# sharckhai/drsa-audio

Measured on AMD Instinct MI355X. Metric: explained samples/sec (LRP+DRSA k=4), higher is better.
Workload: dtype fp32; 1 GPU; GTZAN-128 HeatmapGenerator: LRP (WSquare/Gamma/Epsilon name map) + DRSA subspace heatmaps, K=4 at layer j=7 (conv3 block, d=64), sorted info dict; global_batch=512, per_gpu_batch=512, input=128x128 log-mel, parallelism=data-parallel x1 (no collective on the data path), launch=single process, one_device_rehearsal=False

## Files before the change

### drsa_audio_amd/_capi.py

```python
from __future__ import annotations

import ctypes as C
import os
from typing import Optional

import torch

_HERE = os.path.dirname(os.path.abspath(__file__))
LIB_PATH = os.environ.get("DRSA_AMD_LIB") or os.path.join(_HERE, "lib", "libdrsa_amd.so")

_lib: Optional[C.CDLL] = None

_vp, _fp, _ip = C.c_void_p, C.c_void_p, C.c_void_p
_i64, _i32, _sz, _f32, _f64 = C.c_int64, C.c_int, C.c_size_t, C.c_float, C.c_double

SIGNATURES = {
    "drsa_amd_last_error": (C.c_char_p, []),
    "drsa_amd_version": (_i32, []),
    "drsa_amd_drsa_workspace_bytes": (_sz, [_i64, _i32, _i32]),
    "drsa_amd_drsa_slab_floats": (_sz, [_i32, _i32]),
    "drsa_amd_drsa_partial": (_i32, [_fp, _fp, _i64, _i32, _i32, _fp, _fp, _vp, _sz, _vp]),
    "drsa_amd_drsa_finish": (_i32, [_fp, _i64, _i32, _i32, _fp, _fp, _fp, _i32, _ip, _vp]),
    "drsa_amd_drsa_step": (_i32, [_fp, _fp, _i64, _i32, _i32, _fp, _fp, _fp, _vp, _sz, _vp]),
    "drsa_amd_drsa_fused_supported": (_i32, [_i32, _i32]),
    "drsa_amd_drsa_fused_step": (_i32, [_fp, _fp, _i64, _i32, _i32, _fp, _i64, _fp, _fp, _fp, _fp, _vp, _sz, _vp]),
    "drsa_amd_drsa_fused_step_counted": (_i32, [_fp, _fp, _i64, _i32, _i32, _fp, _i64, _fp, _fp, _fp, _ip, _fp, _vp,
                                                _sz, _vp]),
    "drsa_amd_drsa_finish_counted": (_i32, [_fp, _i64, _i32, _i32, _fp, _fp, _fp, _ip, _vp]),
    "drsa_amd_drsa_coop_status": (_i32, [_vp, _i64, _i32, _i32, _ip, _vp]),
    "drsa_amd_debug_coop_spin_budget": (_i32, [C.c_longlong]),
    "drsa_amd_drsa_objective": (_i32, [_fp, _fp, _i64, _i32, _i32, _fp, _fp, _vp, _sz, _vp]),
    "drsa_amd_drsa_run": (_i32, [_fp, _fp, _i64, _i32, _i32, _fp, _fp, _i32, _fp, _ip, _vp, _sz, _i32, _vp]),
    "drsa_amd_drsa_run_multi": (_i32, [_i32, _vp, _i32, _i32, _vp]),
    "drsa_amd_drsa_run_batched": (_i32, [_i32, _vp, _i32, _i32, _i32, _vp]),
    "drsa_amd_drsa_partial_bf16": (_i32, [_vp, _vp, _i64, _i32, _i32, _fp, _fp, _vp, _sz, _vp]),
    "drsa_amd_drsa_partial_f16": (_i32, [_vp, _vp, _i64, _i32, _i32, _fp, _fp, _vp, _sz, _vp]),
    "drsa_amd_drsa_any_supported": (_i32, [_i32, _i32]),
    "drsa_amd_drsa_any_slab_floats": (_sz, [_i32, _i32]),
    "drsa_amd_drsa_any_workspace_bytes": (_sz, [_i64, _i32, _i32]),
    "drsa_amd_drsa_any_partial": (_i32, [_fp, _fp, _i64, _i32, _i32, _fp, _fp, _vp, _sz, _vp]),
    "drsa_amd_drsa_any_finish": (_i32, [_fp, _i64, _i32, _i32, _fp, _fp, _fp, _i32, _ip, _vp]),
    "drsa_amd_drsa_any_finish_counted": (_i32, [_fp, _i64, _i32, _i32, _fp, _fp, _fp, _ip, _vp]),
    "drsa_amd_drsa_any_step": (_i32, [_fp, _fp, _i64, _i32, _i32, _fp, _fp, _fp, _vp, _sz, _vp]),
    "drsa_amd_drsa_any_objective": (_i32, [_fp, _fp, _i64, _i32, _i32, _fp, _fp, _vp, _sz, _vp]),
    "drsa_amd_drsa_any_run": (_i32, [_fp, _fp, _i64, _i32, _i32, _fp, _fp, _i32, _fp, _ip, _vp, _sz, _i32, _vp]),
    "drsa_amd_polar": (_i32, [_fp, _i32, _fp, _ip, _vp]),
    "drsa_amd_subspace_relevances_workspace_bytes": (_sz, [_i64, _i64, _i32, _i32]),
    "drsa_amd_subspace_relevances": (_i32, [_fp, _fp, _i64, _i64, _i32, _i32, _fp, _fp, _vp, _sz, _vp]),
    "drsa_amd_prca_workspace_bytes": (_sz, [_i64, _i32]),
    "drsa_amd_prca_partial": (_i32, [_fp, _fp, _i64, _i32, _fp, _vp, _sz, _vp]),
    "drsa_amd_prca_finish": (_i32, [_fp, _i64, _i32, _fp, _vp]),
    "drsa_amd_syevj_workspace_bytes": (_sz, [_i32]),
    "drsa_amd_syevj": (_i32, [_fp, _i32, _fp, _fp, _ip, _vp, _sz, _vp]),
    "drsa_amd_conv_weight_floats": (_sz, [_i32, _i32, _i32]),
    "drsa_amd_conv_fwd": (_i32, [_fp, _fp, _fp, _fp, _fp, _vp, _fp, _i32, _i32, _i32, _i32, _i32, _i32, _i32, _vp]),
    "drsa_amd_conv_weight_bf16_elems": (_sz, [_i32, _i32, _i32]),
    "drsa_amd_conv_fwd_has_kernel": (_i32, [_i32, _i32, _i32, _i32, _i32, _i32]),
    "drsa_amd_conv_fwd_bf16": (_i32, [_fp, _vp, _fp, _fp, _fp, _vp, _fp, _i32, _i32, _i32, _i32, _i32, _i32, _i32,
                                      _vp]),
    "drsa_amd_conv_bwd": (_i32, [_fp, _vp, _fp, _fp, _fp, _fp, _i32, _i32, _i32, _i32, _i32, _i32, _i32, _i32,
                                 _i32, _f32, _vp]),
    "drsa_amd_conv_bwd_bf16": (_i32, [_fp, _vp, _vp, _fp, _fp, _fp, _i32, _i32, _i32, _i32, _i32, _i32, _i32, _i32,
                                      _i32, _f32, _vp]),
    "drsa_amd_conv_fwd_den_ring": (_i32, [_fp, _fp, _fp, _fp, _fp, _vp, _fp, _i32, _i32, _i32, _i32, _i32, _vp]),
    "drsa_amd_conv_bwd_den_ring": (_i32, [_fp, _vp, _vp, _i32, _fp, _fp, _fp, _fp, _i32, _i32, _i32, _i32, _i32, _i32,
                                          _i32, _i32, _f32, _vp]),
    "drsa_amd_conv_bwd_den_map": (_i32, [_fp, _vp, _i32, _vp, _i32, _fp, _fp, _fp, _i32, _i32, _i32, _i32, _i32, _i32,
                                         _i32, _i32, _f32, _vp]),
    "drsa_amd_conv_bwd_has_kernel_pw": (_i32, [_i32, _i32, _i32, _i32, _i32]),
    "drsa_amd_conv_bwd_has_kernel_bf16_pw": (_i32, [_i32, _i32, _i32, _i32]),
    "drsa_amd_conv_bwd_bf16_pw": (_i32, [_fp, _vp, _i32, _vp, _fp, _fp, _fp, _i32, _i32, _i32, _i32, _i32, _i32,
                                         _i32, _i32, _f32, _vp]),
    "drsa_amd_conv_bwd_has_kernel_bf16": (_i32, [_i32, _i32, _i32, _i32, _i32]),
    "drsa_amd_convk_supported": (_i32, [_i32, _i32, _i32, _i32]),
    "drsa_amd_convk_weight_floats": (_sz, [_i32, _i32, _i32, _i32, _i32]),
    "drsa_amd_convk_fwd": (_i32, [_fp, _fp, _fp, _fp, _fp, _fp, _i32, _i32, _i32, _i32, _i32, _i32, _i32, _i32, _vp]),
    "drsa_amd_convk_bwd": (_i32, [_fp, _fp, _fp, _fp, _fp, _i32, _i32, _i32, _i32, _i32, _i32, _i32, _i32, _i32,
                                  _i32, _i32, _f32, _vp]),
    "drsa_amd_linear_fwd": (_i32, [_fp, _fp, _fp, _fp, _fp, _i32, _i32, _i32, _vp]),
    "drsa_amd_linear_bwd": (_i32, [_fp, _ip, _i32, _fp, _i32, _i32, _f32, _fp, _fp, _i32, _fp, _i32, _f32, _fp,
                                   _i32, _i32, _i32, _vp]),
    "drsa_amd_linear_rule_fwd": (_i32, [_fp, _fp, _fp, _fp, _fp, _fp, _fp, _fp, _fp, _fp, _fp, _i32, _i32, _i32, _i32,
                                        _vp]),
    "drsa_amd_linear_rule_bwd": (_i32, [_fp, _ip, _i32, _fp, _i32, _fp, _fp, _i32, _i32, _f32, _fp, _fp, _fp, _i32,
                                        _i32, _fp, _i32, _f32, _fp, _i32, _i32, _i32, _vp]),
    "drsa_amd_projection_residual": (_i32, [_fp, _i32, _fp, _vp]),
    "drsa_amd_projection_fwd": (_i32, [_fp, _fp, _fp, _fp, _fp, _fp, _vp, _i32, _i32, _i32, _i32, _i32, _vp]),
    "drsa_amd_projection_bwd": (_i32, [_fp, _vp, _fp, _fp, _fp, _fp, _fp, _fp, _fp, _i32, _i32, _i32, _i32, _i32,
                                       _f32, _f32, _i32, _vp]),
    "drsa_amd_projection_fwd_multi": (_i32, [_fp, _fp, _fp, _ip, _i32, _fp, _fp, _fp, _vp, _i32, _i32, _i32, _i32,
                                             _i32, _vp]),
    "drsa_amd_projection_bwd_multi": (_i32, [_fp, _vp, _fp, _fp, _fp, _fp, _fp, _fp, _ip, _i32, _fp, _i32, _i32, _i32,
                                             _i32, _i32, _f32, _f32, _i32, _vp]),
    "drsa_amd_ab_split": (_i32, [_fp, _fp, _fp, _fp, _fp, _i32, _i32, _i64, _f32, _vp]),
    "drsa_amd_ab_combine": (_i32, [_fp, _fp, _f32, _f32, _fp, _fp, _fp, _i32, _i32, _i64, _i32, _f32, _vp]),
    "drsa_amd_relevance_post": (_i32, [_fp, _fp, _fp, _fp, _i32, _i32, _i64, _i32, _f32, _vp]),
    "drsa_amd_first_layer_bwd": (_i32, [_fp, _vp, _fp, _fp, _i32, _i32, _i32, _i32, _i32, _vp]),
    "drsa_amd_first_layer_den": (_i32, [_fp, _fp, _fp, _i32, _i32, _i32, _i32, _vp]),
    "drsa_amd_first_layer_zbox_maps": (_i32, [_fp, _fp, _fp, _fp, _fp, _fp, _fp, _fp, _i32, _i32, _i32, _vp]),
    "drsa_amd_first_layer_zbox_den": (_i32, [_fp, _vp, _fp, _fp, _fp, _i32, _i32, _i32, _i32, _vp]),
    "drsa_amd_first_layer_zbox_bwd": (_i32, [_fp, _vp, _fp, _fp, _fp, _fp, _fp, _i32, _i32, _i32, _i32, _i32, _vp]),
    "drsa_amd_heatmap_sort": (_i32, [_fp, _i32, _i32, _i32, _i32, _fp, _fp, _fp, _fp, _vp, _vp]),
    "drsa_amd_maxpool_capture": (_i32, [_fp, _fp, _fp, _vp, _fp, _i32, _i32, _i32, _i32, _i32, _i32, _vp]),
    "drsa_amd_relevance_unpool": (_i32, [_fp, _vp, _i32, _i32, _i32, _i32, _i32, _i32, _i32, _fp, _vp]),
    "drsa_amd_avgpool_fwd": (_i32, [_fp, _fp, _i32, _i32, _i32, _i32, _i32, _i32, _vp]),
    "drsa_amd_avgpool_bwd": (_i32, [_fp, _fp, _fp, _fp, _i32, _i32, _f32, _f32, _fp, _fp, _i32, _i32, _i32, _i32,
                                    _i32, _i32, _i32, _vp]),
    "drsa_amd_drsa_vectors": (_i32, [_fp, _fp, _vp, _ip, _i32, _i32, _i32, _i32, _i32, _i32, _i32, _i32, _fp, _fp,
                                     _vp]),
    "drsa_amd_normalize_workspace_bytes": (_sz, []),
    "drsa_amd_normalize_vectors": (_i32, [_fp, _i64, _i32, _fp, _vp, _sz, _vp]),
    "drsa_amd_normalize_sumsq": (_i32, [_fp, _i64, _vp, _sz, _fp, _vp]),
    "drsa_amd_normalize_scale": (_i32, [_fp, _i64, _i32, _fp, _i32, _i64, _fp, _vp]),
    "drsa_amd_logmel_smem_bytes": (_i32, [_i32, _i32, _i32, _i32, _i32]),
    "drsa_amd_logmel": (_i32, [_fp, _i64, _i64, _i32, _i64, _i32, _i32, _i32, _i32, _i32, _i32, _fp, _ip, _ip, _ip,
                               _fp, _i32, _i32, _i32, _f32, _f32, _fp, _vp]),
    "drsa_amd_stft_mel_phase": (_i32, [_fp, _i64, _i64, _i32, _i32, _i32, _i32, _i32, _i32, _i32, _fp, _ip, _ip, _ip,
                                       _fp, _i32, _i32, _fp, _fp, _vp]),
    "drsa_amd_heatmap_mask": (_i32, [_fp, _i64, _i32, _i32, _i32, _i32, _i32, _fp, _i32, _fp, _vp]),
    "drsa_amd_istft_envelope": (_i32, [_fp, _i32, _i32, _i32, _fp]),
    "drsa_amd_mel_to_audio": (_i32, [_fp, _fp, _fp, _i64, _i32, _i32, _i32, _i32, _i32, _i32, _fp, _fp, _fp, _fp,
                                     _vp]),
    "drsa_amd_audio_normalize": (_i32, [_fp, _i64, _i32, _fp, _i64, _i32, _i32, _vp]),
    "drsa_amd_mel_relevance_to_stft": (_i32, [_fp, _fp, _fp, _i64, _i32, _i32, _i32, _i32, _ip, _ip, _ip, _fp, _i32,
                                              _f32, _fp, _vp]),
    "drsa_amd_heatmap_mask_large": (_i32, [_fp, _i64, _i32, _i32, _i32, _i32, _i32, _fp, _i32, _fp, _vp]),
    "drsa_amd_stft_mask_to_audio": (_i32, [_fp, _fp, _i64, _i32, _i32, _i32, _i32, _fp, _fp, _fp, _vp]),
}

class DrsaProblem(C.Structure):
    _fields_ = [("A", _vp), ("C", _vp), ("N", _i64), ("d", _i32), ("K", _i32), ("U_io", _vp), ("U_tmp", _vp),
                ("f_traj", _vp), ("counter", _vp), ("ws", _vp), ("ws_size", _sz), ("dtype", _i32)]


DRSA_OK, DRSA_EINVAL, DRSA_EWORKSPACE, DRSA_EUNSUPPORTED, DRSA_ETIMEOUT = 0, -1, -2, -3, -4

XM_NONE, XM_MUL, XM_SPLIT = 0, 1, 2
POST_NONE, POST_DIV, POST_MASK, POST_DIV_RING = 0, 1, 2, 3
POST_DIV_MAP = 4


class DrsaAmdError(RuntimeError):
    pass


def load(path: str = LIB_PATH) -> C.CDLL:
    global _lib
    if _lib is not None:
        return _lib
    if not os.path.exists(path):
        raise DrsaAmdError(
            f"drsa_amd HIP library not found at {path}; build it with "
            f"`python -m drsa_audio_amd.build` (hipcc, gfx950). There is no CPU fallback.")
    lib = C.CDLL(path)
    for name, (res, args) in SIGNATURES.items():
        fn = getattr(lib, name)
        fn.restype = res
        fn.argtypes = args
    _lib = lib
    return lib


def lib() -> C.CDLL:
    return _lib if _lib is not None else load()


def check(rc: int, what: str = "") -> None:
    if rc != 0:
        msg = lib().drsa_amd_last_error().decode(errors="replace")
        raise DrsaAmdError(f"{what or 'drsa_amd'} failed (rc={rc}): {msg}")


def require_gpu(t: torch.Tensor, name: str, dtype=torch.float32) -> None:
    if not isinstance(t, torch.Tensor):
        raise DrsaAmdError(f"{name}: expected a torch.Tensor on the GPU, got {type(t).__name__}")
    if not t.is_cuda:
        raise DrsaAmdError(f"{name}: tensor must live on the GPU (HIP device); got {t.device}. "
                           "drsa_audio_amd has no CPU path.")
    if dtype is not None and t.dtype != dtype:
        raise DrsaAmdError(f"{name}: expected {dtype}, got {t.dtype}")
    if not t.is_contiguous():
        raise DrsaAmdError(f"{name}: tensor must be contiguous")


def ptr(t: Optional[torch.Tensor]) -> Optional[int]:
    return None if t is None else t.data_ptr()


def stream_ptr(device: Optional[torch.device] = None) -> int:
    return torch.cuda.current_stream(device).cuda_stream


def call(name: str, *args) -> None:
    fn = getattr(lib(), name)
    check(fn(*args), name)
```

### drsa_audio_amd/csrc/conv_bwd_b.hip

```cpp
#include "lrp_conv_inst.h"

#ifndef DRSA_CONV_CIC_BWD32
#define DRSA_CONV_CIC_BWD32 8
#endif
#ifndef DRSA_CONV_CIC_BWD64_32
#define DRSA_CONV_CIC_BWD64_32 8
#endif

CONV_TABLE(kTableBwdB,
    BWD_SET(64, 32, DRSA_CONV_CIC_BWD64_32),
    BWD_SET(32, 32, DRSA_CONV_CIC_BWD32))

#ifdef DRSA_CONV_STAMP
extern "C" int drsa_amd_debug_conv_stamps(void* buf) {
  return (int)hipMemcpyToSymbol(HIP_SYMBOL(drsa_conv::g_conv_stamps), &buf, sizeof(buf));
}
#endif
```

### drsa_audio_amd/csrc/lrp_conv.hip

```cpp
#include "common.h"
#include "lrp_conv.h"
#include "lrp_conv_table.h"

#include <stdlib.h>

#define DRSA_CONV_TABLES(X) \
  X(FwdA) X(FwdB) X(FwdC) X(FwdD) X(FwdE) X(BwdA) X(BwdB) X(BwdC) X(FwdBfA) X(FwdBfB) X(FwdBfC) X(FwdP4) X(BwdBfA) X(BwdBfB)

namespace drsa_conv {
#define DRSA_CONV_DECLARE(T) extern const Table kTable##T;
DRSA_CONV_TABLES(DRSA_CONV_DECLARE)
extern const Table kTableSmall;
}

namespace {
using drsa_conv::Entry;
using namespace drsa_conv;

#define DRSA_CONV_ADDRESS(T) &drsa_conv::kTable##T,
const drsa_conv::Table* kTables[] = {DRSA_CONV_TABLES(DRSA_CONV_ADDRESS)};

int pad32(int c) { return (c + 31) / 32 * 32; }

const Entry* find(int cin_p, int cout_p, int W, int ng, int amode, int epi, int et = 0, int pw = 2) {
  const int wide = W >= kWideW;
  for (const drsa_conv::Table* t : kTables)
    for (int i = 0; i < t->n; ++i) {
      const Entry& e = t->entries[i];
      if (e.cin_p == cin_p && e.cout_p == cout_p && e.ng == ng && e.amode == amode && e.epi == epi && e.et == et &&
          e.pw == pw && e.wide == wide)
        return &e;
    }
  return nullptr;
}

#ifndef DRSA_CONV_SMALL_WG
#define DRSA_CONV_SMALL_WG 512
#endif
const Entry* small_tile(const Entry* e, int H, int W, int batch) {
  if (e->th != 8 || e->tw != 8) return e;
  if ((int64_t)((H + 7) / 8) * ((W + 7) / 8) * batch >= DRSA_CONV_SMALL_WG) return e;
  for (int i = 0; i < drsa_conv::kTableSmall.n; ++i) {
    const Entry& c = drsa_conv::kTableSmall.entries[i];
    if (c.cin_p == e->cin_p && c.cout_p == e->cout_p && c.ng == e->ng && c.amode == e->amode && c.epi == e->epi &&
        c.et == e->et && c.pw == e->pw)
      return &c;
  }
  return e;
}

int launch(const Entry* e0, const ConvArgs& args, int batch, hipStream_t s) {
  DRSA_REQUIRE((int64_t)(args.cin > args.cout ? args.cin : args.cout) * args.H * args.W < ((int64_t)1 << 31),
               "conv: one sample's channels x H x W must stay below 2^31");
  const Entry* e = small_tile(e0, args.H, args.W, batch);
  DRSA_SMEM(e->fn, e->lds);
  const int tiles = ((args.H + e->th - 1) / e->th) * ((args.W + e->tw - 1) / e->tw);
  hipLaunchKernelGGL(e->fn, dim3(tiles, batch), dim3(kThreads), e->lds, s, args);
  DRSA_LAUNCH_CHECK();
  return DRSA_OK;
}

int cin_pad(int cin) { return cin == 1 ? 1 : pad32(cin); }

const Entry* find_fwd(int cin, int cout, int W, int ng, int pool, int bf16) {
  return find(bf16 ? pad32(cin) : cin_pad(cin), pad32(cout), W, ng, A_DENSE, pool ? EPI_FWD_POOL : EPI_FWD_RELU,
              bf16 ? 1 : 0, pool == 2 ? 4 : 2);
}

const Entry* find_bwd(int cin, int cout, int W, int ng, int sparse, int bf16, int pool_w) {
  return find(pad32(cin), pad32(cout), W, ng, sparse ? A_POOLSPARSE : A_DENSE, EPI_BWD, bf16 ? 1 : 0, pool_w);
}

int no_kernel(const char* entry, int cin, int cout, int W, int ng, int sparse, int bf16, const char* pool_key, int pool) {
  drsa::set_error("%s: no kernel for cin=%d cout=%d W=%d ng=%d sparse=%d bf16=%d %s=%d", entry, cin, cout, W, ng, sparse,
                  bf16 ? 1 : 0, pool_key, pool);
  return DRSA_EUNSUPPORTED;
}

struct FwdCall {
  const char* name;
  const float* in;
  const void* wts;
  int bf16;
  const float *bias, *den_map;
  float* out;
  uint8_t* out_amax;
  float* out_den;
  int den_ring_only;
  int B, cin, cout, H, W, ng, pool;
};

int conv_fwd_run(const FwdCall& c, void* stream) {
  const char* n = c.name;
  DRSA_REQUIRE(c.B > 0 && c.H > 0 && c.W > 0, "%s: bad shape", n);
  DRSA_REQUIRE(!c.bf16 || c.cin > 1, "%s: cin = 1 runs on drsa_amd_conv_fwd (fp32 VALU kernel)", n);
  DRSA_REQUIRE(c.ng >= 1 && c.ng <= 3, "%s: ng must be 1..3", n);
  DRSA_REQUIRE(c.H % 2 == 0 && c.W % 2 == 0, "%s: H and W must be even (got %dx%d)", n, c.H, c.W);
  DRSA_REQUIRE(c.pool >= 0 && c.pool <= 2, "%s: pool must be 0 (none), 1 (2x2) or 2 (2x4)", n);
  DRSA_REQUIRE(!c.pool || c.out_amax, "%s: pool needs out_amax", n);
  DRSA_REQUIRE(c.pool || c.W % 4 == 0, "%s: an unpooled output needs W %% 4 == 0 (float4 epilogue; got W=%d)", n, c.W);
  DRSA_REQUIRE(c.pool != 2 || c.W % 4 == 0, "%s: a 2x4 pool needs W %% 4 == 0 (got W=%d)", n, c.W);
  DRSA_REQUIRE(!c.bf16 || ((uintptr_t)c.wts & 15) == 0, "%s: weights must be 16-byte aligned", n);
  ConvArgs a{};
  a.in = c.in; a.wts = reinterpret_cast<const float*>(c.wts); a.bias = c.bias; a.den_map = c.den_map; a.out = c.out;
  a.out_amax = c.out_amax; a.out_den = c.out_den; a.H = c.H; a.W = c.W; a.cin = c.cin; a.cout = c.cout; a.clones = 1;
  a.den_ring_only = c.den_ring_only;
  if (c.cin == 1 && c.pool == 1 && c.W % 8 == 0)
    return drsa_first_conv_pool(a, pad32(c.cout), c.ng, c.B, (hipStream_t)stream);
  const Entry* e = find_fwd(c.cin, c.cout, c.W, c.ng, c.pool, c.bf16);
  if (!e) return no_kernel(n, c.cin, c.cout, c.W, c.ng, 0, c.bf16, "pool", c.pool);
  return launch(e, a, c.B, (hipStream_t)stream);
}

struct BwdCall {
  const char* name;
  const float* g;
  const uint8_t* g_amax;
  int pool_w;
  const void* wts;
  int bf16;
  const float *x, *den, *den_const4;
  int den_shared;
  float* out;
  int Bq, clones, cin, cout, H, W, ng, xmode, post;
  float eps;
};

int conv_bwd_run(const BwdCall& c, void* stream) {
  const char* n = c.name;
  DRSA_REQUIRE(c.Bq > 0 && c.clones > 0 && c.Bq % c.clones == 0, "%s: bad batch/clones", n);
  if (c.bf16) {
    DRSA_REQUIRE(c.ng == 1, "%s: bf16 weights need ng == 1 (the Gamma x-/W- term is for the fp32 first layer)", n);
    DRSA_REQUIRE(c.cin >= 16, "%s: bf16 weights need cin >= 16 (16-channel bf16 chunks)", n);
    DRSA_REQUIRE(((uintptr_t)c.wts & 15) == 0, "%s: bf16 weights must be 16-byte aligned", n);
  } else {
    DRSA_REQUIRE(c.ng >= 1 && c.ng <= 2, "%s: ng must be 1..2", n);
  }
  DRSA_REQUIRE(c.den_const4 || (c.H % 2 == 0 && c.W % 4 == 0),
               "%s: H must be even and W %% 4 == 0 (got %dx%d)", n, c.H, c.W);
  DRSA_REQUIRE(c.xmode == XM_NONE || c.x, "%s: xmode needs x", n);
  DRSA_REQUIRE(c.post == POST_NONE || (c.x && (c.den || c.post == POST_MASK)), "%s: POST_DIV needs x and den", n);
  const int sparse = c.g_amax != nullptr;
  const Entry* e = find_bwd(c.cin, c.cout, c.W, c.ng, sparse, c.bf16, c.pool_w);
  if (!e) return no_kernel(n, c.cin, c.cout, c.W, c.ng, sparse, c.bf16, "pool_w", c.pool_w);
  ConvArgs a{};
  a.in = c.g; a.in_amax = c.g_amax; a.wts = reinterpret_cast<const float*>(c.wts); a.x = c.x; a.den = c.den;
  a.den_const4 = c.den_const4; a.den_shared = c.den_shared; a.out = c.out; a.H = c.H; a.W = c.W; a.cin = c.cin;
  a.cout = c.cout; a.clones = c.clones; a.xmode = c.xmode; a.post = c.post; a.eps = c.eps;
  return launch(e, a, c.Bq, (hipStream_t)stream);
}

}

extern "C" {

size_t drsa_amd_conv_weight_floats(int cin, int cout, int ng) {
  return (size_t)ng * 9 * cin_pad(cin) * pad32(cout);
}

size_t drsa_amd_conv_weight_bf16_elems(int cin, int cout, int ng) {
  return (size_t)ng * 9 * pad32(cin) * pad32(cout);
}

int drsa_amd_conv_fwd_has_kernel(int cin, int cout, int W, int ng, int pool, int bf16) {
  if (cin == 1 && !bf16 && pool == 1) return 1;
  if (pool < 0 || pool > 2 || ng < 1 || ng > 3 || (bf16 && cin == 1)) return 0;
  return find_fwd(cin, cout, W, ng, pool, bf16) != nullptr;
}

int drsa_amd_conv_bwd_has_kernel_bf16(int cin, int cout, int W, int ng, int sparse) {
  if (cin < 16 || ng != 1) return 0;
  return find_bwd(cin, cout, W, ng, sparse, 1, 2) != nullptr;
}

int drsa_amd_conv_bwd_has_kernel_pw(int cin, int cout, int W, int ng, int pool_w) {
  if (cin < 2 || (pool_w != 2 && pool_w != 4) || (pool_w == 4 && (W / 4) % 4 != 0)) return 0;
  return find_bwd(cin, cout, W, ng, 1, 0, pool_w) != nullptr;
}

int drsa_amd_conv_bwd_has_kernel_bf16_pw(int cin, int cout, int W, int pool_w) {
  if (cin < 16 || (pool_w != 2 && pool_w != 4)) return 0;
  return find_bwd(cin, cout, W, 1, 1, 1, pool_w) != nullptr;
}

int drsa_amd_conv_fwd(const float* in, const float* wts, const float* bias, const float* den_map, float* out,
                      uint8_t* out_amax, float* out_den, int B, int cin, int cout, int H, int W, int ng,
                      int pool, void* stream) {
  return conv_fwd_run({"conv_fwd", in, wts, 0, bias, den_map, out, out_amax, out_den, 0, B, cin, cout, H, W, ng, pool},
                      stream);
}

int drsa_amd_conv_fwd_bf16(const float* in, const uint16_t* wts, const float* bias, const float* den_map, float* out,
                           uint8_t* out_amax, float* out_den, int B, int cin, int cout, int H, int W, int ng,
                           int pool, void* stream) {
  return conv_fwd_run({"conv_fwd_bf16", in, wts, 1, bias, den_map, out, out_amax, out_den, 0, B, cin, cout, H, W, ng, pool},
                      stream);
}

int drsa_amd_conv_fwd_den_ring(const float* in, const float* wts, const float* bias, const float* den_map, float* out,
                               uint8_t* out_amax, float* den_ring, int B, int cout, int H, int W, int ng,
                               void* stream) {
  DRSA_REQUIRE(in && wts && den_map && out && out_amax && den_ring, "conv_fwd_den_ring: null pointer");
  DRSA_REQUIRE(B > 0 && H >= 4 && W > 0 && H % 2 == 0 && W % 16 == 0,
               "conv_fwd_den_ring: needs H >= 4 even and W %% 16 == 0 (got %dx%d)", H, W);
  return conv_fwd_run({"conv_fwd_den_ring", in, wts, 0, bias, den_map, out, out_amax, den_ring, 1, B, 1, cout, H, W, ng, 1},
                      stream);
}

int drsa_amd_conv_bwd(const float* g, const uint8_t* g_amax, const float* wts, const float* x, const float* den,
                      float* out, int Bq, int clones, int cin, int cout, int H, int W, int ng, int xmode,
                      int post, float eps, void* stream) {
  return conv_bwd_run({"conv_bwd", g, g_amax, 2, wts, 0, x, den, nullptr, 0, out, Bq, clones, cin, cout, H, W, ng, xmode,
                       post, eps}, stream);
}

int drsa_amd_conv_bwd_bf16(const float* g, const uint8_t* g_amax, const uint16_t* wts, const float* x, const float* den,
                           float* out, int Bq, int clones, int cin, int cout, int H, int W, int ng, int xmode,
                           int post, float eps, void* stream) {
  return conv_bwd_run({"conv_bwd_bf16", g, g_amax, 2, wts, 1, x, den, nullptr, 0, out, Bq, clones, cin, cout, H, W, ng,
                       xmode, post, eps}, stream);
}

int drsa_amd_conv_bwd_bf16_pw(const float* g, const uint8_t* g_amax, int pool_w, const uint16_t* wts, const float* x,
                              const float* den, float* out, int Bq, int clones, int cin, int cout, int H, int W,
                              int xmode, int post, float eps, void* stream) {
  DRSA_REQUIRE(g_amax && (pool_w == 2 || pool_w == 4), "conv_bwd_bf16_pw: needs g_amax and pool_w 2 or 4");
  return conv_bwd_run({"conv_bwd_bf16_pw", g, g_amax, pool_w, wts, 1, x, den, nullptr, 0, out, Bq, clones, cin, cout, H,
                       W, 1, xmode, post, eps}, stream);
}

int drsa_amd_conv_bwd_den_map(const float* g, const uint8_t* g_amax, int pool_w, const void* wts, int wts_bf16,
                              const float* x, const float* den_map, float* out, int Bq, int clones, int cin, int cout,
                              int H, int W, int ng, int xmode, float eps, void* stream) {
  DRSA_REQUIRE(x && den_map, "conv_bwd_den_map: needs x and den_map");
  DRSA_REQUIRE(!g_amax || pool_w == 2 || pool_w == 4, "conv_bwd_den_map: pool_w must be 2 or 4");
  DRSA_REQUIRE(xmode == XM_NONE || xmode == XM_MUL || xmode == XM_SPLIT, "conv_bwd_den_map: bad xmode");
  const bool pool24 = g_amax && pool_w == 4;
  DRSA_REQUIRE(wts_bf16 || !pool24 || ng == 1, "conv_bwd_den_map: fp32 weights need ng 1 under a 2x4 pool (got ng=%d)", ng);
  DRSA_REQUIRE(!pool24 || (W / 4) % 4 == 0, "conv_bwd_den_map: a 2x4 pool-sparse g needs W / 4 %% 4 == 0 (got W=%d)", W);
  return conv_bwd_run({"conv_bwd_den_map", g, g_amax, g_amax ? pool_w : 2, wts, wts_bf16 != 0, x, den_map, nullptr, 1, out,
                       Bq, clones, cin, cout, H, W, ng, xmode, POST_DIV, eps}, stream);
}

int drsa_amd_conv_bwd_den_ring(const float* g, const uint8_t* g_amax, const void* wts, int wts_bf16, const float* x,
                               const float* den_ring, const float* den_const4, float* out, int Bq, int clones, int cin,
                               int cout, int H, int W, int ng, int xmode, float eps, void* stream) {
  DRSA_REQUIRE(x && den_ring && den_const4, "conv_bwd_den_ring: needs x, den_ring and den_const4");
  DRSA_REQUIRE(H >= 2 && W >= 8 && W % 8 == 0,
               "conv_bwd_den_ring: needs pooled H >= 2 and W >= 8, W %% 8 == 0 (got %dx%d)", H, W);
  DRSA_REQUIRE(xmode == XM_NONE || xmode == XM_MUL || xmode == XM_SPLIT, "conv_bwd_den_ring: bad xmode");
  DRSA_REQUIRE(((uintptr_t)den_const4 & 15) == 0, "conv_bwd_den_ring: den_const4 must be 16-byte aligned");
  return conv_bwd_run({"conv_bwd_den_ring", g, g_amax, 2, wts, wts_bf16 != 0, x, den_ring, den_const4, 0, out, Bq, clones,
                       cin, cout, H, W, ng, xmode, POST_DIV_RING, eps}, stream);
}

}
```

### drsa_audio_amd/csrc/lrp_conv_config.h

```cpp
#pragma once
#include <stddef.h>

#ifndef DRSA_CONV_PD_BWD
#define DRSA_CONV_PD_BWD 2
#endif
#ifndef DRSA_CONV_BWD_ES
#define DRSA_CONV_BWD_ES 1
#endif
#ifndef DRSA_CONV_BWD_WPE
#define DRSA_CONV_BWD_WPE 3
#endif
#ifndef DRSA_CONV_PIN_SMALL
#define DRSA_CONV_PIN_SMALL 1
#endif
#ifndef DRSA_CONV_PD_SMALL
#define DRSA_CONV_PD_SMALL 3
#endif
#ifndef DRSA_CONV_SMALL_WPE
#define DRSA_CONV_SMALL_WPE 4
#endif
#ifndef DRSA_CONV_SMALL_ES
#define DRSA_CONV_SMALL_ES 2
#endif
#ifndef DRSA_CONV_PRE_D
#define DRSA_CONV_PRE_D 0
#endif
#ifndef DRSA_CONV_PRE_N
#define DRSA_CONV_PRE_N 64
#endif
#ifndef DRSA_CONV_BF_WPE
#define DRSA_CONV_BF_WPE 2
#endif
#ifndef DRSA_CONV_FWD_WPE_128
#define DRSA_CONV_FWD_WPE_128 3
#endif
#ifndef DRSA_CONV_FWD_WPE_WIDE
#define DRSA_CONV_FWD_WPE_WIDE 3
#endif
#ifndef DRSA_CONV_FWD_WPE
#define DRSA_CONV_FWD_WPE 3
#endif
#ifndef DRSA_CONV_FWD128_TW
#define DRSA_CONV_FWD128_TW 8
#endif

namespace drsa_conv {

constexpr int kThreads = 256;

template <int V, int M>
constexpr int round_up() { return (V + M - 1) / M * M; }

constexpr int halo_stride(int hx, int mw) {
  int r = hx;
  const int want = (mw == 8) ? 16 : 8;
  while (r % 32 != want) ++r;
  return r;
}

enum AMode { A_DENSE = 0, A_POOLSPARSE = 1 };
enum Epi { EPI_FWD_POOL = 0, EPI_FWD_RELU = 1, EPI_BWD = 2 };

constexpr int kWideW = 32;
constexpr int wide_tile_w(int epi, int et, int cin_p, int cout_p, int fwd128_tw = DRSA_CONV_FWD128_TW) {
  if (et != 0) return 32;
  if (epi != EPI_BWD) return cout_p == 128 ? fwd128_tw : cout_p == 64 ? 16 : 32;
  return (cout_p == 64 && cin_p <= 128) || cout_p == 128 ? 16 : 32;
}
constexpr int tile_mw(int tw) { return tw == 8 ? 4 : 8; }

constexpr int XO = 3;

constexpr int bf_stride(int hx) {
  int r = hx;
  while (r % 16 != 8) ++r;
  return r;
}

template <int CIN, int COUT, int TH, int TW, int MW, int CIC, int NG, int AMODE, int EPI, int ET = 0, int PW = 2>
struct ConvCfg {
  static constexpr int CIN_ = CIN, COUT_ = COUT, TH_ = TH, TW_ = TW, MW_ = MW, CIC_ = CIC, NG_ = NG;
  static constexpr int AMODE_ = AMODE, EPI_ = EPI;
  static constexpr bool BF = ET == 1;
  static constexpr int HY = TH + 2, HX = TW + 2;
  static constexpr int HXB = bf_stride(HX);
  static constexpr size_t bf_halo_floats = (size_t)2 * HY * HXB * 4;
  static constexpr size_t bf_w_floats = (size_t)NG * 9 * 2 * COUT * 4;
  static constexpr int RS = halo_stride(HX + XO, MW);
  static constexpr int PLANE_RAW = HY * RS;
  static constexpr int PLANE = PLANE_RAW + ((PLANE_RAW % 32) == 0 ? 4 : 0);
  static constexpr int MTW = 2 * MW;
  static constexpr int MTH = 32 / MTW;
  static constexpr int MTX = TW / MTW;
  static constexpr int MT = (TH / MTH) * MTX;
  static constexpr int NT = COUT / 32;
  static constexpr int WM = MT >= 4 ? 4 : MT;
  static constexpr int WN = (4 / WM) < NT ? (4 / WM) : NT;
  static constexpr int MPW = MT / WM;
  static constexpr int NPW = NT / WN;
  static constexpr int KC = 9 * CIC;
  static constexpr int KCP = round_up<KC, 2>();
  static constexpr int NCHUNK = CIN / CIC;
  static constexpr int TWP = (TW == 32) ? 48 : TW;
  static constexpr bool SMALL_BWD = EPI == EPI_BWD && NG == 1 && CIC <= 8 && COUT <= 32;
  static constexpr int ES = (EPI == EPI_BWD && WN == 1) ? (SMALL_BWD ? DRSA_CONV_SMALL_ES : DRSA_CONV_BWD_ES) : 1;
  static constexpr int TCH = WN * 32 / ES;
  static constexpr size_t staging_floats =
      BF ? bf_halo_floats + bf_w_floats : (size_t)CIC * PLANE + (size_t)NG * KCP * COUT;
  static constexpr size_t epi_floats = (size_t)TCH * TH * TWP;
  static constexpr size_t lds_floats = staging_floats > epi_floats ? staging_floats : epi_floats;
  static constexpr int WPE = BF ? (COUT <= 64 ? DRSA_CONV_BF_WPE : 1)
                             : (EPI == EPI_BWD && NG == 1) ? (SMALL_BWD ? DRSA_CONV_SMALL_WPE : DRSA_CONV_BWD_WPE)
                             : (EPI != EPI_BWD && CIC <= 8 && COUT <= 32 && NG <= 2 ? DRSA_CONV_FWD_WPE
                                : EPI != EPI_BWD && CIC <= 8 && NG <= 2 && COUT == 64 ? DRSA_CONV_FWD_WPE_WIDE
                                : EPI != EPI_BWD && CIC <= 4 && NG <= 2 && COUT == 128 && TW == 8 ? DRSA_CONV_FWD_WPE_128 : 1);
  static constexpr bool PIN = SMALL_BWD && DRSA_CONV_PIN_SMALL;
  static constexpr int PD = PIN ? DRSA_CONV_PD_SMALL : DRSA_CONV_PD_BWD > 0 && EPI >= EPI_BWD ? DRSA_CONV_PD_BWD : 1;
  static_assert(TH % MTH == 0 && TW % MTW == 0, "tile must be a multiple of the M-tile");
  static_assert(COUT % 32 == 0, "COUT must be padded to 32");
  static_assert(CIN % CIC == 0, "CIN must be a multiple of the chunk");
  static_assert(MT % WM == 0 && NT % WN == 0 && WM * WN <= 4, "wave split");
  static_assert(!BF || (CIC == 16 && (EPI < EPI_BWD ? AMODE == A_DENSE : EPI == EPI_BWD)),
                "bf16: 16-channel chunks; dense forward, or the per-clone backward (dense or pool-sparse g)");
  static_assert(PW == 2 || (PW == 4 && (EPI == EPI_FWD_POOL || (EPI == EPI_BWD && AMODE == A_POOLSPARSE &&
                                                                  (ET == 1 || TW % 16 == 0)))),
                "2x4 pool windows: the forward pool epilogue, or the backward's pool-sparse staging (fp32: "
                "tiles of whole float4 cell groups)");
  static constexpr int PW_ = PW;
};

}
```

### drsa_audio_amd/csrc/lrp_conv_inst.h

```cpp
#pragma once
#include "lrp_conv_kernel.h"
#include "lrp_conv_table.h"

namespace drsa_conv {

template <int... P>
constexpr Entry conv_entry(int wide) {
  static_assert(sizeof...(P) == 11, "CONV_ENTRY takes every ConvCfg parameter");
  constexpr int p[] = {P...};
  return Entry{p[0], p[1], p[2], p[3], p[4], p[5], p[6], p[7], p[8],
               conv3x3_kernel<P...>, ConvCfg<P...>::lds_floats * sizeof(float), p[9], p[10], wide};
}
#define CONV_ENTRY(CIN, COUT, TH, TW, MW, CIC, NG, AM, EP, ET, PW) \
  drsa_conv::conv_entry<CIN, COUT, TH, TW, MW, CIC, NG, AM, EP, ET, PW>(0)
#define CONV_ENTRY_WIDE(CIN, COUT, TH, TW, MW, CIC, NG, AM, EP, ET, PW) \
  drsa_conv::conv_entry<CIN, COUT, TH, TW, MW, CIC, NG, AM, EP, ET, PW>(1)

#define CONV_FAMILY(CIN, COUT, CIC, NG, AM, EP, ET, PW)                                             \
  CONV_ENTRY_WIDE(CIN, COUT, 8, drsa_conv::wide_tile_w(EP, ET, CIN, COUT),                          \
                  drsa_conv::tile_mw(drsa_conv::wide_tile_w(EP, ET, CIN, COUT)), CIC, NG, AM, EP, ET, PW), \
  CONV_ENTRY(CIN, COUT, 8, 8, 4, CIC, NG, AM, EP, ET, PW)

#define FWD_SET_ET(CIN, COUT, CIC, ET)                                                      \
  CONV_FAMILY(CIN, COUT, CIC, 1, drsa_conv::A_DENSE, drsa_conv::EPI_FWD_POOL, ET, 2),        \
  CONV_FAMILY(CIN, COUT, CIC, 2, drsa_conv::A_DENSE, drsa_conv::EPI_FWD_POOL, ET, 2),        \
  CONV_FAMILY(CIN, COUT, CIC, 3, drsa_conv::A_DENSE, drsa_conv::EPI_FWD_POOL, ET, 2),        \
  CONV_FAMILY(CIN, COUT, CIC, 1, drsa_conv::A_DENSE, drsa_conv::EPI_FWD_RELU, ET, 2),        \
  CONV_FAMILY(CIN, COUT, CIC, 2, drsa_conv::A_DENSE, drsa_conv::EPI_FWD_RELU, ET, 2),        \
  CONV_FAMILY(CIN, COUT, CIC, 3, drsa_conv::A_DENSE, drsa_conv::EPI_FWD_RELU, ET, 2)
#define FWD_SET(CIN, COUT, CIC) FWD_SET_ET(CIN, COUT, CIC, 0)
#define FWD_SET_BF(CIN, COUT) FWD_SET_ET(CIN, COUT, 16, 1)

#define FWD_SET_P4(CIN, COUT, CIC, ET)                                                      \
  CONV_FAMILY(CIN, COUT, CIC, 1, drsa_conv::A_DENSE, drsa_conv::EPI_FWD_POOL, ET, 4),        \
  CONV_FAMILY(CIN, COUT, CIC, 2, drsa_conv::A_DENSE, drsa_conv::EPI_FWD_POOL, ET, 4),        \
  CONV_FAMILY(CIN, COUT, CIC, 3, drsa_conv::A_DENSE, drsa_conv::EPI_FWD_POOL, ET, 4)

#define BWD_SET(CIN, COUT, CIC)                                                             \
  CONV_FAMILY(CIN, COUT, CIC, 1, drsa_conv::A_DENSE, drsa_conv::EPI_BWD, 0, 2),              \
  CONV_FAMILY(CIN, COUT, CIC, 2, drsa_conv::A_DENSE, drsa_conv::EPI_BWD, 0, 2),              \
  CONV_FAMILY(CIN, COUT, CIC, 1, drsa_conv::A_POOLSPARSE, drsa_conv::EPI_BWD, 0, 2),         \
  CONV_FAMILY(CIN, COUT, CIC, 2, drsa_conv::A_POOLSPARSE, drsa_conv::EPI_BWD, 0, 2)

#define BWD_SET_BF(CIN, COUT)                                                               \
  CONV_FAMILY(CIN, COUT, 16, 1, drsa_conv::A_DENSE, drsa_conv::EPI_BWD, 1, 2),               \
  CONV_FAMILY(CIN, COUT, 16, 1, drsa_conv::A_POOLSPARSE, drsa_conv::EPI_BWD, 1, 2)
#define BWD_SET_BF_P4(CIN, COUT) CONV_FAMILY(CIN, COUT, 16, 1, drsa_conv::A_POOLSPARSE, drsa_conv::EPI_BWD, 1, 4)

#define CONV_TABLE(NAME, ...)                                                                     \
  namespace drsa_conv {                                                                           \
  static const Entry NAME##_e[] = {__VA_ARGS__};                                                  \
  extern const Table NAME = {NAME##_e, (int)(sizeof(NAME##_e) / sizeof(NAME##_e[0]))};            \
  }

}
```

### drsa_audio_amd/csrc/lrp_conv_kernel.h

```cpp
#pragma once
#include "common.h"
#include "lrp_conv.h"
#include "lrp_conv_config.h"
#include "lrp_conv_mfma.h"
#include "lrp_conv_stage.h"
#include "lrp_conv_stage_bf.h"

#include <type_traits>

namespace drsa_conv {

#ifdef DRSA_CONV_STAMP
static __device__ unsigned long long* g_conv_stamps;
#endif

__device__ const float g_zero_bias3[3 * 128] = {};

template <int CIN, int COUT, int TH, int TW, int MW, int CIC, int NG, int AMODE, int EPI, int ET = 0, int PW = 2>
__global__ __launch_bounds__(kThreads) __attribute__((amdgpu_waves_per_eu(ConvCfg<CIN, COUT, TH, TW, MW, CIC, NG, AMODE, EPI, ET, PW>::WPE))) void conv3x3_kernel(ConvArgs a) {
  using Cfg = ConvCfg<CIN, COUT, TH, TW, MW, CIC, NG, AMODE, EPI, ET, PW>;
  constexpr int HY = Cfg::HY, HX = Cfg::HX, RS = Cfg::RS, PLANE = Cfg::PLANE;
  constexpr int MTH = Cfg::MTH, MTW = Cfg::MTW, MTX = Cfg::MTX;
  constexpr int WM = Cfg::WM, MPW = Cfg::MPW, NPW = Cfg::NPW;
  constexpr int KC = Cfg::KC, KCP = Cfg::KCP;

  extern __shared__ __attribute__((aligned(16))) float smem[];
#ifdef DRSA_CONV_STAMP
  constexpr bool kStamp = EPI == EPI_BWD && CIN == 32 && COUT == 32 && AMODE == A_POOLSPARSE && ET == 0;
  unsigned long long* const stp = kStamp && g_conv_stamps && threadIdx.x == 0
                                      ? g_conv_stamps + ((size_t)blockIdx.y * gridDim.x + blockIdx.x) * 16 : nullptr;
#define CONV_STAMP(slot) do { if (stp) stp[(slot)] = __builtin_amdgcn_s_memtime(); } while (0)
#else
#define CONV_STAMP(slot) do {} while (0)
#endif
  CONV_STAMP(0);
  float* halo = smem;
  float* wl = smem + (Cfg::BF ? Cfg::bf_halo_floats : (size_t)CIC * PLANE);

  const int tid = threadIdx.x, lane = lane_id(), w = wave_id();
  const int H = a.H, W = a.W;
  const int tiles_x = (W + TW - 1) / TW;
  const int tile_id = blockIdx.x, bq = blockIdx.y;
  const int ty0 = (tile_id / tiles_x) * TH;
  const int tx0 = (tile_id % tiles_x) * TW;
  const int bs = bq / a.clones;
  const int wm = w % WM, wn = w / WM;
  const bool active = w < WM * Cfg::WN;
  const int h = lane >> 5;

  int pix_off[MPW], pix_y[MPW], pix_x[MPW];
#pragma unroll
  for (int u = 0; u < MPW; ++u) {
    const int mt = wm * MPW + u;
    const int p = lane & 31, win = p >> 2, sub = p & 3;
    pix_y[u] = (mt / MTX) * MTH + 2 * (win / MW) + (sub >> 1);
    pix_x[u] = (mt % MTX) * MTW + 2 * (win % MW) + (sub & 1);
    pix_off[u] = Cfg::BF ? (h * HY + pix_y[u]) * Cfg::HXB + pix_x[u] : pix_y[u] * RS + pix_x[u] + XO;
  }

  f32x16 acc[NG][MPW][NPW];
#pragma unroll
  for (int g = 0; g < NG; ++g)
#pragma unroll
    for (int u = 0; u < MPW; ++u)
#pragma unroll
      for (int v = 0; v < NPW; ++v)
#pragma unroll
        for (int r = 0; r < 16; ++r) acc[g][u][v][r] = 0.f;

  constexpr int TWP = Cfg::TWP, TCH = Cfg::TCH;
  constexpr int NV4 = TCH * TH * TW / 4;
  constexpr int V4T = (NV4 + kThreads - 1) / kThreads;
  constexpr int NCELL = TCH * (TH / 2) * (TW / 2);
  constexpr int CT = (NCELL + kThreads - 1) / kThreads;
  float* T = smem;
  constexpr int ES = Cfg::ES;
  static_assert(ES == 1 || ES == 2 || ES == 4, "epilogue split must be 1, 2 or 4");
  auto stage = [&](int v, auto valfn, int sub = 0) {
    __syncthreads();
    if (active) {
#pragma unroll
      for (int u = 0; u < MPW; ++u)
#pragma unroll
        for (int r = 0; r < 16; ++r) {
          const int cf = (r & 3) + 8 * (r >> 2) + 4 * h;
          if constexpr (ES == 1) {
            T[((wn * 32 + cf) * TH + pix_y[u]) * TWP + pix_x[u]] = valfn(u, r);
          } else {
            if ((r >> (ES == 2 ? 3 : 2)) == sub) T[((cf - TCH * sub) * TH + pix_y[u]) * TWP + pix_x[u]] = valfn(u, r);
          }
        }
    }
    __syncthreads();
  };
  auto gch = [&](int cl, int v) { return ((cl >> 5) * NPW + v) * 32 + (cl & 31); };
  auto gchs = [&](int cl, int v, int sub) { return ES == 1 ? gch(cl, v) : v * 32 + sub * TCH + cl; };
  typename std::conditional<Cfg::BF, StagerBF<Cfg>, Stager<Cfg>>::type stg;
  stg.load(a, 0, tid, ty0, tx0, bq, bs);
  CONV_STAMP(11);
  for (int chunk = 0; chunk + (EPI == EPI_BWD ? 1 : 0) < Cfg::NCHUNK; ++chunk) {
    __syncthreads();
    if (chunk == 0) CONV_STAMP(9);
    if constexpr (Cfg::BF) stg.store(halo, wl, tid, ty0, tx0);
    else stg.store(halo, wl, tid);
    if (chunk == 0) CONV_STAMP(10);
    __syncthreads();
    CONV_STAMP(1 + 2 * chunk);
    if (chunk + 1 < Cfg::NCHUNK) stg.load(a, (chunk + 1) * CIC, tid, ty0, tx0, bq, bs);
    if (!active) continue;
    if constexpr (Cfg::BF)
      mfma_chunk_bf<Cfg>(reinterpret_cast<const uint4*>(halo), reinterpret_cast<const uint4*>(wl), pix_off, lane, wn, acc);
    else
      mfma_chunk<Cfg, Cfg::PD>(halo, wl, pix_off, lane, wn, acc);
    CONV_STAMP(2 + 2 * chunk);
  }
  constexpr int Q = TH * TW / 4, CS = kThreads / Q;
  static_assert(kThreads % Q == 0, "float4 groups per tile must divide the block");
  const int cl0 = tid / Q, rem = tid % Q;
  const int py = rem / (TW / 4), px = (rem % (TW / 4)) * 4;
  const bool pix_ok = ty0 + py < H && tx0 + px < W;
  const int HW = H * W;
  const size_t pix = pix_ok ? (size_t)(ty0 + py) * W + tx0 + px : 0;
  const float* xs = a.x ? a.x + (size_t)bs * a.cout * HW + pix : nullptr;
  const float* ds = a.den ? a.den + (a.den_shared ? (size_t)0 : (size_t)bs * a.cout * HW) + pix : nullptr;
  float* oqp = a.out + (size_t)bq * a.cout * HW + pix;
  const bool need_x = a.xmode != XM_NONE || a.post != POST_NONE;
  const bool mul_x = a.xmode != XM_NONE, split_x = a.xmode == XM_SPLIT;
  const bool ring = a.post == POST_DIV_RING && a.den_const4;
  const bool post_div = a.post == POST_DIV || ring, post_any = a.post != POST_NONE;
  const float* xsrc = xs ? xs : oqp;
  const float* dsrc = (ds && post_div && !ring) ? ds : xsrc;
  const float eps = a.eps;
  const bool on_ring = !pix_ok || ty0 + py == 0 || ty0 + py == H - 1 || tx0 + px == 0 || tx0 + px + 4 >= W;
  const bool use_c4 = ring && !on_ring;
  const int ring_n = 2 * W + 8 * (H - 2);
  const int Y = ty0 + py, X = tx0 + px;
  const int ring_i = !pix_ok ? 0 : Y == 0 ? X : Y == H - 1 ? W + X : 2 * W + (Y - 1) * 8 + (X == 0 ? 0 : 4);
  const float* rsrc = ring ? a.den + (size_t)bs * a.cout * ring_n + ring_i : dsrc;
  const size_t dstride = ring ? (size_t)ring_n : (size_t)HW;
  const unsigned upix = (unsigned)pix;
  float* const obase = a.out + (size_t)bq * a.cout * HW;
  const float* const xbase = a.x ? a.x + (size_t)bs * a.cout * HW : obase;
  auto epi_loads = [&](int v, int sub, float4 (&xk)[V4T], float4 (&dk)[V4T], bool lx = true, bool ld = true,
                       int i0 = 0, int i1 = -1) {
    if (i1 < 0) i1 = V4T;
#pragma unroll
    for (int it = i0; it < i1; ++it) {
      const int cl = cl0 + it * CS;
      const int co = gchs(cl, v, sub);
      const bool ok = cl < TCH && co < a.cout;
      const int coc = ok ? co : 0;
      if (lx) xk[it] = *reinterpret_cast<const float4*>(xbase + (upix + (unsigned)coc * (unsigned)HW));
      if (ld) dk[it] = *reinterpret_cast<const float4*>(use_c4 ? a.den_const4 + (size_t)coc * 4 : rsrc + coc * dstride);
    }
  };
  constexpr int kPreN = DRSA_CONV_PRE_N < V4T ? DRSA_CONV_PRE_N : V4T;
  float4 pre_x[V4T], pre_d[V4T];
  if constexpr (EPI == EPI_BWD) {
    __syncthreads();
    if constexpr (Cfg::BF) stg.store(halo, wl, tid, ty0, tx0);
    else stg.store(halo, wl, tid);
    __syncthreads();
    CONV_STAMP(2 * Cfg::NCHUNK - 1);
    epi_loads(0, 0, pre_x, pre_d, true, DRSA_CONV_PRE_D, 0, kPreN);

    if (active) {
      if constexpr (Cfg::BF)
        mfma_chunk_bf<Cfg>(reinterpret_cast<const uint4*>(halo), reinterpret_cast<const uint4*>(wl), pix_off, lane, wn,
                           acc);
      else
        mfma_chunk<Cfg, Cfg::PD>(halo, wl, pix_off, lane, wn, acc);
    }
    CONV_STAMP(2 * Cfg::NCHUNK);
  }

  auto pool_cells = [&](auto pwc, auto&& fn) {
    constexpr int PWc = decltype(pwc)::value;
    constexpr int CW = TW / PWc, NC = TCH * (TH / 2) * CW;
    const int H2 = H >> 1, W2 = W / PWc;
#pragma unroll
    for (int it = 0; it < CT; ++it) {
      const int i = tid + it * kThreads;
      if (i < NC) {
        const int cl = i / ((TH / 2) * CW), rem = i % ((TH / 2) * CW);
        const int cy = rem / CW, cx = rem % CW;
        fn(it, cl, cy, cx, (ty0 >> 1) + cy, tx0 / PWc + cx, H2, W2);
      }
    }
  };
#pragma unroll
  for (int v = 0; v < NPW; ++v) {
    if constexpr (EPI == EPI_FWD_POOL || EPI == EPI_FWD_RELU) {
      const float* bb = a.bias ? a.bias : g_zero_bias3;
      float b0[16], b1[16], b2[16];
#pragma unroll
      for (int r = 0; r < 16; ++r) {
        const int co = gch(wn * 32 + (r & 3) + 8 * (r >> 2) + 4 * h, v);
        const bool cok = co < a.cout;
        const float x0 = bb[co], x1 = bb[COUT + co], x2 = bb[2 * COUT + co];
        b0[r] = cok ? x0 : 0.f;
        b1[r] = cok ? x1 : 0.f;
        b2[r] = cok ? x2 : 0.f;
      }
      stage(v, [&](int u, int r) {
        const float z = acc[0][u][v][r] + b0[r];
        float y = z > 0.f ? z : 0.f;
        if (z != z) y = z;
        return y;
      });
      int am_keep[CT];
      if constexpr (EPI == EPI_FWD_POOL) {
        auto pass0 = [&](auto pwc) {
          constexpr int PWc = decltype(pwc)::value;
          pool_cells(pwc, [&](int it, int cl, int cy, int cx, int qy, int qx, int H2, int W2) {
            const int co = gch(cl, v);
            const float* t = T + (cl * TH + 2 * cy) * TWP + PWc * cx;
            int am = 0;
            float m = t[0];
#pragma unroll
            for (int s4 = 1; s4 < 2 * PWc; ++s4) {
              const float yv = t[(s4 / PWc) * TWP + s4 % PWc];
              if (yv > m || (yv != yv && m == m)) { m = yv; am = s4; }
            }
            am_keep[it] = am;
            if (co < a.cout && qy < H2 && qx < W2) {
              const size_t o = (size_t)bq * a.cout * H2 * W2 + (unsigned)((co * H2 + qy) * W2 + qx);
              a.out[o] = m;
              a.out_amax[o] = (uint8_t)am;
            }
          });
        };
        if constexpr (PW == 4) {
#pragma unroll
          for (int it = 0; it < CT; ++it) am_keep[it] = 0;
          pass0(std::integral_constant<int, 4>{});
        } else {
          const int H2 = H >> 1, W2 = W >> 1;
#pragma unroll
          for (int it = 0; it < CT; ++it) {
            const int i = tid + it * kThreads;
            am_keep[it] = 0;
            if (i < NCELL) {
              const int cl = i / ((TH / 2) * (TW / 2)), rem = i % ((TH / 2) * (TW / 2));
              const int cy = rem / (TW / 2), cx = rem % (TW / 2);
              const int co = gch(cl, v);
              const int qy = (ty0 >> 1) + cy, qx = (tx0 >> 1) + cx;
              const float* t = T + (cl * TH + 2 * cy) * TWP + 2 * cx;
              const float yy[4] = {t[0], t[1], t[TWP], t[TWP + 1]};
              int am = 0;
              float m = yy[0];
#pragma unroll
              for (int s4 = 1; s4 < 4; ++s4)
                if (yy[s4] > m || (yy[s4] != yy[s4] && m == m)) { m = yy[s4]; am = s4; }
              am_keep[it] = am;
              if (co < a.cout && qy < H2 && qx < W2) {
                const size_t o = (size_t)bq * a.cout * H2 * W2 + (unsigned)((co * H2 + qy) * W2 + qx);
                a.out[o] = m;
                a.out_amax[o] = (uint8_t)am;
              }
            }
          }
        }
      } else {
#pragma unroll
        for (int it = 0; it < V4T; ++it) {
          const int i = tid + it * kThreads;
          if (i < NV4) {
            const int cl = i / (TH * TW / 4), rem = i % (TH * TW / 4);
            const int py = rem / (TW / 4), px = (rem % (TW / 4)) * 4;
            const int co = gch(cl, v);
            if (co < a.cout && ty0 + py < H && tx0 + px < W) {
              const float4 val = *reinterpret_cast<const float4*>(T + (cl * TH + py) * TWP + px);
              *reinterpret_cast<float4*>(a.out + (size_t)bq * a.cout * H * W + (unsigned)((co * H + ty0 + py) * W + tx0 + px)) = val;
            }
          }
        }
      }
      if (a.out_den && a.den_map) {
        if constexpr (EPI == EPI_FWD_POOL) {
          auto gather_map = [&](auto pwc) {
            constexpr int PWc = decltype(pwc)::value;
            pool_cells(pwc, [&](int it, int cl, int, int, int qy, int qx, int H2, int W2) {
              const int co = gch(cl, v);
              const int am = am_keep[it];
              if (co < a.cout && qy < H2 && qx < W2)
                a.out_den[(size_t)bq * a.cout * H2 * W2 + (unsigned)((co * H2 + qy) * W2 + qx)] =
                    a.den_map[(unsigned)((co * H + 2 * qy + am / PWc) * W + PWc * qx + am % PWc)];
            });
          };
          if constexpr (PW == 4) {
            gather_map(std::integral_constant<int, 4>{});
          } else {
            const int H2 = H >> 1, W2 = W >> 1;
#pragma unroll
            for (int it = 0; it < CT; ++it) {
              const int i = tid + it * kThreads;
              if (i < NCELL) {
                const int cl = i / ((TH / 2) * (TW / 2)), rem = i % ((TH / 2) * (TW / 2));
                const int cy = rem / (TW / 2), cx = rem % (TW / 2);
                const int co = gch(cl, v);
                const int qy = (ty0 >> 1) + cy, qx = (tx0 >> 1) + cx;
                const int am = am_keep[it];
                if (co < a.cout && qy < H2 && qx < W2)
                  a.out_den[(size_t)bq * a.cout * H2 * W2 + (unsigned)((co * H2 + qy) * W2 + qx)] =
                      a.den_map[(unsigned)((co * H + 2 * qy + (am >> 1)) * W + 2 * qx + (am & 1))];
              }
            }
          }
        } else {
#pragma unroll
          for (int it = 0; it < V4T; ++it) {
            const int i = tid + it * kThreads;
            if (i < NV4) {
              const int cl = i / (TH * TW / 4), rem = i % (TH * TW / 4);
              const int py = rem / (TW / 4), px = (rem % (TW / 4)) * 4;
              const int co = gch(cl, v);
              if (co < a.cout && ty0 + py < H && tx0 + px < W)
                *reinterpret_cast<float4*>(a.out_den + (size_t)bq * a.cout * H * W + (unsigned)((co * H + ty0 + py) * W + tx0 + px)) =
                    *reinterpret_cast<const float4*>(a.den_map + (unsigned)((co * H + ty0 + py) * W + tx0 + px));
            }
          }
        }
      } else if (a.out_den) {
        stage(v, [&](int u, int r) {
          if constexpr (NG >= 2) {
            const float z0 = acc[1][u][v][r] + b1[r];
            float z1 = b2[r];
            if constexpr (NG == 3) z1 = acc[2][u][v][r] + b2[r];
            return z0 + z1;
          }
          return acc[0][u][v][r] + b1[r];
        });
        if constexpr (EPI == EPI_FWD_POOL) {
          auto gather_den = [&](auto pwc) {
            constexpr int PWc = decltype(pwc)::value;
            pool_cells(pwc, [&](int it, int cl, int cy, int cx, int qy, int qx, int H2, int W2) {
              const int co = gch(cl, v);
              const int am = am_keep[it];
              if (co < a.cout && qy < H2 && qx < W2)
                a.out_den[(size_t)bq * a.cout * H2 * W2 + (unsigned)((co * H2 + qy) * W2 + qx)] =
                    T[(cl * TH + 2 * cy + am / PWc) * TWP + PWc * cx + am % PWc];
            });
          };
          if constexpr (PW == 4) {
            gather_den(std::integral_constant<int, 4>{});
          } else {
            const int H2 = H >> 1, W2 = W >> 1;
#pragma unroll
            for (int it = 0; it < CT; ++it) {
              const int i = tid + it * kThreads;
              if (i < NCELL) {
                const int cl = i / ((TH / 2) * (TW / 2)), rem = i % ((TH / 2) * (TW / 2));
                const int cy = rem / (TW / 2), cx = rem % (TW / 2);
                const int co = gch(cl, v);
                const int qy = (ty0 >> 1) + cy, qx = (tx0 >> 1) + cx;
                const int am = am_keep[it];
                if (co < a.cout && qy < H2 && qx < W2)
                  a.out_den[(size_t)bq * a.cout * H2 * W2 + (unsigned)((co * H2 + qy) * W2 + qx)] =
                      T[(cl * TH + 2 * cy + (am >> 1)) * TWP + 2 * cx + (am & 1)];
              }
            }
          }
        } else {
#pragma unroll
          for (int it = 0; it < V4T; ++it) {
            const int i = tid + it * kThreads;
            if (i < NV4) {
              const int cl = i / (TH * TW / 4), rem = i % (TH * TW / 4);
              const int py = rem / (TW / 4), px = (rem % (TW / 4)) * 4;
              const int co = gch(cl, v);
              if (co < a.cout && ty0 + py < H && tx0 + px < W) {
                const float4 val = *reinterpret_cast<const float4*>(T + (cl * TH + py) * TWP + px);
                *reinterpret_cast<float4*>(a.out_den + (size_t)bq * a.cout * H * W + (unsigned)((co * H + ty0 + py) * W + tx0 + px)) = val;
              }
            }
          }
        }
      }
    } else {
#pragma unroll
     for (int sub = 0; sub < ES; ++sub) {
      float4 Rk[V4T], xk[V4T], dk[V4T];
      if (v == 0 && sub == 0) {
#pragma unroll
        for (int it = 0; it < kPreN; ++it) xk[it] = pre_x[it];
        epi_loads(v, sub, xk, dk, true, false, kPreN, V4T);
        if (DRSA_CONV_PRE_D) {
#pragma unroll
          for (int it = 0; it < V4T; ++it) dk[it] = pre_d[it];
        } else {
          epi_loads(v, sub, xk, dk, false, true);
        }
      } else {
        epi_loads(v, sub, xk, dk);
      }
      stage(v, [&](int u, int r) { return acc[0][u][v][r]; }, sub);
      if (NG == 1 && a.xmode == XM_MUL && post_div) {
#pragma unroll
        for (int it = 0; it < V4T; ++it) {
          const int cl = cl0 + it * CS;
          const int co = gchs(cl, v, sub);
          const bool ok = cl < TCH && co < a.cout;
          const int clc = ok ? cl : 0, coc = ok ? co : 0;
          const float4 t = *reinterpret_cast<const float4*>(T + (clc * TH + py) * TWP + px);
          const float4 x = xk[it], d = dk[it];
          auto f = [&](float tt, float xx, float dd) {
            const float q = div_nb(xx * tt, stab(dd, eps));
            return (xx > 0.f) ? q : 0.f;
          };
          const float4 R = make_float4(f(t.x, x.x, d.x), f(t.y, x.y, d.y), f(t.z, x.z, d.z), f(t.w, x.w, d.w));
          if (ok && pix_ok) *reinterpret_cast<float4*>(obase + (upix + (unsigned)coc * (unsigned)HW)) = R;
        }
        continue;
      }
#pragma unroll
      for (int it = 0; it < V4T; ++it) {
        const int cl = cl0 + it * CS;
        const int co = gchs(cl, v, sub);
        const int clc = (cl < TCH && co < a.cout) ? cl : 0;
        const float4 t = *reinterpret_cast<const float4*>(T + (clc * TH + py) * TWP + px);
        if (!need_x) xk[it] = make_float4(0.f, 0.f, 0.f, 0.f);
        const float4 x = xk[it];
        auto xm = [&](float xx) { const float m = split_x ? fmaxf(xx, 0.f) : xx; return mul_x ? m : 1.f; };
        Rk[it] = make_float4(xm(x.x) * t.x, xm(x.y) * t.y, xm(x.z) * t.z, xm(x.w) * t.w);
      }
      if constexpr (NG >= 2) {
        if (split_x) {
          stage(v, [&](int u, int r) { return acc[1][u][v][r]; }, sub);
#pragma unroll
          for (int it = 0; it < V4T; ++it) {
            const int cl = cl0 + it * CS;
            const int co = gchs(cl, v, sub);
            const int clc = (cl < TCH && co < a.cout) ? cl : 0;
            const float4 t = *reinterpret_cast<const float4*>(T + (clc * TH + py) * TWP + px);
            const float4 x = xk[it];
            Rk[it].x += fminf(x.x, 0.f) * t.x;
            Rk[it].y += fminf(x.y, 0.f) * t.y;
            Rk[it].z += fminf(x.z, 0.f) * t.z;
            Rk[it].w += fminf(x.w, 0.f) * t.w;
          }
        }
      }
#pragma unroll
      for (int it = 0; it < V4T; ++it) {
        const int cl = cl0 + it * CS;
        const int co = gchs(cl, v, sub);
        const bool ok = cl < TCH && co < a.cout;
        const int coc = ok ? co : 0;
        float4 R = Rk[it];
        const float4 x = xk[it], d = dk[it];
        auto post = [&](float rr, float xx, float dd) {
          const float q = div_nb(rr, stab(dd, eps));
          const float y = post_div ? q : rr;
          return (post_any && !(xx > 0.f)) ? 0.f : y;
        };
        R = make_float4(post(R.x, x.x, d.x), post(R.y, x.y, d.y), post(R.z, x.z, d.z), post(R.w, x.w, d.w));
        if (ok && pix_ok) *reinterpret_cast<float4*>(obase + (upix + (unsigned)coc * (unsigned)HW)) = R;
      }
     }
    }
  }
#ifdef DRSA_CONV_STAMP
  if (stp) {
    stp[13] = __builtin_amdgcn_s_memtime();
    stp[14] = (unsigned long long)__builtin_amdgcn_s_getreg(4 | (31 << 11));
    stp[15] = (unsigned long long)__builtin_amdgcn_s_getreg(20 | (31 << 11));
  }
#endif
#undef CONV_STAMP
}

}
```

### drsa_audio_amd/csrc/lrp_conv_stage.h

```cpp
#pragma once
#include "common.h"
#include "lrp_conv.h"
#include "lrp_conv_config.h"

namespace drsa_conv {

template <class Cfg, int NT_ = kThreads>
struct Stager {
  static constexpr int CIN = Cfg::CIN_, COUT = Cfg::COUT_, TH = Cfg::TH_, TW = Cfg::TW_, CIC = Cfg::CIC_;
  static constexpr int NG = Cfg::NG_, HY = Cfg::HY, HX = Cfg::HX, RS = Cfg::RS, PLANE = Cfg::PLANE;
  static constexpr int KC = Cfg::KC, KCP = Cfg::KCP;
  static constexpr bool DENSE = Cfg::AMODE_ == A_DENSE;
  static constexpr int Q4 = TW / 4, DROWS = CIC * HY;
  static constexpr int DI = (DROWS * Q4 + NT_ - 1) / NT_, DH = (DROWS * 2 + NT_ - 1) / NT_;
  static constexpr int CY = TH / 2 + 2, CX = TW / 2 + 2, Q8 = TW / 8 > 0 ? TW / 8 : 1, SROWS = CIC * CY;
  static constexpr int SI = (SROWS * Q8 + NT_ - 1) / NT_, SH = (SROWS * 2 + NT_ - 1) / NT_;
  static constexpr bool P4 = !DENSE && Cfg::PW_ == 4;
  static constexpr int Q16 = TW / 16 > 0 ? TW / 16 : 1;
  static constexpr int SI4 = (SROWS * Q16 + NT_ - 1) / NT_;
  static constexpr int NI = DENSE ? DI : P4 ? SI4 : SI, NH = DENSE ? DH : SH;
  static constexpr int NWV = NG * KCP * (COUT / 4), WIT = (NWV + NT_ - 1) / NT_;
  float4 st_i[NI];
  uint32_t st_ia[DENSE ? 1 : NI];
  float st_h[NH];
  int st_ha[DENSE ? 1 : NH];
  float4 st_w[WIT];

  __device__ __forceinline__ void load(const ConvArgs& a, int c0, int tid, int ty0, int tx0, int bq, int bs) {
    const int H = a.H, W = a.W, H2 = H >> 1, W2 = W >> 1;
    const int W4 = W >> 2;
    const float* __restrict__ inb = a.in + (size_t)bq * a.cin * (DENSE ? H * W : H2 * (P4 ? W4 : W2));
    const uint8_t* __restrict__ amb = DENSE ? nullptr : a.in_amax + (size_t)bs * a.cin * H2 * (P4 ? W4 : W2);
    if constexpr (P4) {
      const int qy0 = (ty0 >> 1) - 1, cx0 = tx0 >> 2;
#pragma unroll
      for (int it = 0; it < SI4; ++it) {
        const int i = tid + it * NT_;
        const int row = i / Q16, q = i % Q16;
        const int ci = row / CY, ry = row % CY;
        const int cy = qy0 + ry, cx = cx0 + 4 * q, c = c0 + ci;
        const bool ok = i < SROWS * Q16 && cy >= 0 && cy < H2 && c < a.cin && cx < W4;
        const int o = ok ? (c * H2 + cy) * W4 + cx : 0;
        const float4 v = *reinterpret_cast<const float4*>(inb + o);
        const uint32_t am = *reinterpret_cast<const uint32_t*>(amb + o);
        st_i[it] = ok ? v : make_float4(0.f, 0.f, 0.f, 0.f);
        st_ia[it] = ok ? am : 0xffffffffu;
      }
#pragma unroll
      for (int it = 0; it < SH; ++it) {
        const int i = tid + it * NT_;
        const int row = i >> 1, side = i & 1;
        const int ci = row / CY, ry = row % CY;
        const int cy = qy0 + ry, cx = side ? cx0 + TW / 4 : cx0 - 1, c = c0 + ci;
        const bool ok = i < SROWS * 2 && cy >= 0 && cy < H2 && cx >= 0 && cx < W4 && c < a.cin;
        const int o = ok ? (c * H2 + cy) * W4 + cx : 0;
        const float v = inb[o];
        const int am = (int)amb[o];
        st_h[it] = ok ? v : 0.f;
        st_ha[it] = ok ? am : 0xff;
      }
    } else if constexpr (DENSE) {
      if ((W & 3) == 0) {
#pragma unroll
        for (int it = 0; it < DI; ++it) {
          const int i = tid + it * NT_;
          const int row = i / Q4, q = i % Q4;
          const int ci = row / HY, hy = row % HY;
          const int gy = ty0 - 1 + hy, gx = tx0 + 4 * q, c = c0 + ci;
          const bool ok = i < DROWS * Q4 && gy >= 0 && gy < H && c < a.cin && gx < W;
          const int o = ok ? (c * H + gy) * W + gx : 0;
          const float4 v = *reinterpret_cast<const float4*>(inb + o);
          st_i[it] = ok ? v : make_float4(0.f, 0.f, 0.f, 0.f);
        }
      } else {
#pragma unroll
        for (int it = 0; it < DI; ++it) {
          const int i = tid + it * NT_;
          const int row = i / Q4, q = i % Q4;
          const int ci = row / HY, hy = row % HY;
          const int gy = ty0 - 1 + hy, gx = tx0 + 4 * q, c = c0 + ci;
          const bool rok = i < DROWS * Q4 && gy >= 0 && gy < H && c < a.cin;
          float vv[4];
#pragma unroll
          for (int e = 0; e < 4; ++e) {
            const bool ok = rok && gx + e < W;
            const int o = ok ? (c * H + gy) * W + gx + e : 0;
            const float v = inb[o];
            vv[e] = ok ? v : 0.f;
          }
          st_i[it] = make_float4(vv[0], vv[1], vv[2], vv[3]);
        }
      }
#pragma unroll
      for (int it = 0; it < DH; ++it) {
        const int i = tid + it * NT_;
        const int row = i >> 1, side = i & 1;
        const int ci = row / HY, hy = row % HY;
        const int gy = ty0 - 1 + hy, gx = side ? tx0 + TW : tx0 - 1, c = c0 + ci;
        const bool ok = i < DROWS * 2 && gy >= 0 && gy < H && gx >= 0 && gx < W && c < a.cin;
        const int o = ok ? (c * H + gy) * W + gx : 0;
        const float v = inb[o];
        st_h[it] = ok ? v : 0.f;
      }
    } else {
      const int qy0 = (ty0 >> 1) - 1, qx0 = (tx0 >> 1) - 1;
      if ((W2 & 3) == 0) {
#pragma unroll
        for (int it = 0; it < SI; ++it) {
          const int i = tid + it * NT_;
          const int row = i / Q8, q = i % Q8;
          const int ci = row / CY, ry = row % CY;
          const int cy = qy0 + ry, cx = qx0 + 1 + 4 * q, c = c0 + ci;
          const bool ok = i < SROWS * Q8 && 4 * q < TW / 2 && cy >= 0 && cy < H2 && c < a.cin && cx < W2;
          const int o = ok ? (c * H2 + cy) * W2 + cx : 0;
          const float4 v = *reinterpret_cast<const float4*>(inb + o);
          const uint32_t am = *reinterpret_cast<const uint32_t*>(amb + o);
          st_i[it] = ok ? v : make_float4(0.f, 0.f, 0.f, 0.f);
          st_ia[it] = ok ? am : 0x04040404u;
        }
      } else {
#pragma unroll
        for (int it = 0; it < SI; ++it) {
          const int i = tid + it * NT_;
          const int row = i / Q8, q = i % Q8;
          const int ci = row / CY, ry = row % CY;
          const int cy = qy0 + ry, cx = qx0 + 1 + 4 * q, c = c0 + ci;
          const bool rok = i < SROWS * Q8 && 4 * q < TW / 2 && cy >= 0 && cy < H2 && c < a.cin;
          float vv[4];
          uint32_t aa = 0;
#pragma unroll
          for (int e = 0; e < 4; ++e) {
            const bool ok = rok && cx + e < W2 && 4 * q + e < TW / 2;
            const int o = ok ? (c * H2 + cy) * W2 + cx + e : 0;
            const float v = inb[o];
            const uint32_t am = amb[o];
            vv[e] = ok ? v : 0.f;
            aa |= (ok ? am : 4u) << (8 * e);
          }
          st_i[it] = make_float4(vv[0], vv[1], vv[2], vv[3]);
          st_ia[it] = aa;
        }
      }
#pragma unroll
      for (int it = 0; it < SH; ++it) {
        const int i = tid + it * NT_;
        const int row = i >> 1, side = i & 1;
        const int ci = row / CY, ry = row % CY;
        const int cy = qy0 + ry, cx = side ? qx0 + CX - 1 : qx0, c = c0 + ci;
        const bool ok = i < SROWS * 2 && cy >= 0 && cy < H2 && cx >= 0 && cx < W2 && c < a.cin;
        const int o = ok ? (c * H2 + cy) * W2 + cx : 0;
        const float v = inb[o];
        const int am = (int)amb[o];
        st_h[it] = ok ? v : 0.f;
        st_ha[it] = ok ? am : 4;
      }
    }
#pragma unroll
    for (int it = 0; it < WIT; ++it) {
      const int idx = tid + it * NT_;
      const int g = idx / (KCP * (COUT / 4)), rem = idx % (KCP * (COUT / 4));
      const int k = rem / (COUT / 4), c4 = (rem % (COUT / 4)) * 4;
      const bool ok = idx < NWV && k < KC;
      const float4 v = *reinterpret_cast<const float4*>(a.wts + (ok ? ((size_t)g * 9 * CIN + c0 * 9 + k) * COUT + c4 : 0));
      st_w[it] = ok ? v : make_float4(0.f, 0.f, 0.f, 0.f);
    }
  }

  __device__ __forceinline__ static void put_cell(float* halo, int ci, int ry, int rx, float v, int sb) {
    float* d = halo + ci * PLANE + (2 * ry - 1) * RS + 2 * rx - 1 + XO;
    if (ry > 0) *reinterpret_cast<float2*>(d) = make_float2(sb == 0 ? v : 0.f, sb == 1 ? v : 0.f);
    if (ry < CY - 1) *reinterpret_cast<float2*>(d + RS) = make_float2(sb == 2 ? v : 0.f, sb == 3 ? v : 0.f);
  }

  __device__ __forceinline__ static void put_cell4(float* halo, int ci, int ry, int rx, float v, int sb) {
    float* d = halo + ci * PLANE + (2 * ry - 1) * RS + 4 * rx;
    if (ry > 0)
      *reinterpret_cast<float4*>(d) = make_float4(sb == 0 ? v : 0.f, sb == 1 ? v : 0.f, sb == 2 ? v : 0.f, sb == 3 ? v : 0.f);
    if (ry < CY - 1)
      *reinterpret_cast<float4*>(d + RS) =
          make_float4(sb == 4 ? v : 0.f, sb == 5 ? v : 0.f, sb == 6 ? v : 0.f, sb == 7 ? v : 0.f);
  }

  __device__ __forceinline__ void store(float* halo, float* wl, int tid) const {
    if constexpr (P4) {
      static_assert(XO == 3, "P4 cells land on 16-byte aligned columns 4 rx");
#pragma unroll
      for (int it = 0; it < SI4; ++it) {
        const int i = tid + it * NT_;
        if (i < SROWS * Q16) {
          const int row = i / Q16, q = i % Q16;
          const int ci = row / CY, ry = row % CY;
          const float vv[4] = {st_i[it].x, st_i[it].y, st_i[it].z, st_i[it].w};
#pragma unroll
          for (int e = 0; e < 4; ++e)
            put_cell4(halo, ci, ry, 1 + 4 * q + e, vv[e], (int)((st_ia[it] >> (8 * e)) & 0xffu));
        }
      }
#pragma unroll
      for (int it = 0; it < SH; ++it) {
        const int i = tid + it * NT_;
        if (i < SROWS * 2) {
          const int row = i >> 1, side = i & 1;
          put_cell4(halo, row / CY, row % CY, side ? TW / 4 + 1 : 0, st_h[it], st_ha[it]);
        }
      }
    } else if constexpr (DENSE) {
#pragma unroll
      for (int it = 0; it < DI; ++it) {
        const int i = tid + it * NT_;
        if (i < DROWS * Q4) {
          const int row = i / Q4, q = i % Q4;
          const int ci = row / HY, hy = row % HY;
          *reinterpret_cast<float4*>(halo + ci * PLANE + hy * RS + 1 + XO + 4 * q) = st_i[it];
        }
      }
#pragma unroll
      for (int it = 0; it < DH; ++it) {
        const int i = tid + it * NT_;
        if (i < DROWS * 2) {
          const int row = i >> 1, side = i & 1;
          const int ci = row / HY, hy = row % HY;
          halo[ci * PLANE + hy * RS + (side ? HX - 1 : 0) + XO] = st_h[it];
        }
      }
    } else {
#pragma unroll
      for (int it = 0; it < SI; ++it) {
        const int i = tid + it * NT_;
        const int q = i % Q8;
        if (i < SROWS * Q8 && 4 * q < TW / 2) {
          const int row = i / Q8;
          const int ci = row / CY, ry = row % CY;
          const float vv[4] = {st_i[it].x, st_i[it].y, st_i[it].z, st_i[it].w};
#pragma unroll
          for (int e = 0; e < 4; ++e)
            if (4 * q + e < TW / 2) put_cell(halo, ci, ry, 1 + 4 * q + e, vv[e], (int)((st_ia[it] >> (8 * e)) & 0xffu));
        }
      }
#pragma unroll
      for (int it = 0; it < SH; ++it) {
        const int i = tid + it * NT_;
        if (i < SROWS * 2) {
          const int row = i >> 1, side = i & 1;
          put_cell(halo, row / CY, row % CY, side ? CX - 1 : 0, st_h[it], st_ha[it]);
        }
      }
    }
#pragma unroll
    for (int it = 0; it < WIT; ++it) {
      const int idx = tid + it * NT_;
      if (idx < NWV) *reinterpret_cast<float4*>(wl + (size_t)idx * 4) = st_w[it];
    }
  }
};

}
```

### drsa_audio_amd/csrc/lrp_conv_table.h

```cpp
#pragma once
#include "lrp_conv.h"
#include "lrp_conv_config.h"

namespace drsa_conv {

typedef void (*KernFn)(ConvArgs);

struct Entry {
  int cin_p, cout_p, th, tw, mw, cic, ng, amode, epi;
  KernFn fn;
  size_t lds;
  int et = 0;
  int pw = 2;
  int wide = 0;
};

struct Table {
  const Entry* entries;
  int n;
};

}
```

### include/drsa_amd.h

```cpp
#ifndef DRSA_AMD_H
#define DRSA_AMD_H

#include <stddef.h>
#include <stdint.h>

#ifdef __cplusplus
extern "C" {
#endif

#define DRSA_OK 0
#define DRSA_EINVAL (-1)
#define DRSA_EWORKSPACE (-2)
#define DRSA_EUNSUPPORTED (-3)
#define DRSA_ETIMEOUT (-4)

const char* drsa_amd_last_error(void);
int drsa_amd_version(void);


size_t drsa_amd_drsa_workspace_bytes(int64_t N, int d, int K);

size_t drsa_amd_drsa_slab_floats(int d, int K);

int drsa_amd_drsa_partial(const float* A, const float* C, int64_t N, int d, int K, const float* U,
                          float* gs_out, void* workspace, size_t workspace_bytes, void* stream);

int drsa_amd_drsa_finish(const float* gs, int64_t N_total, int d, int K, const float* U, float* U_out,
                         float* f_out, int objective_only, int* iters_out, void* stream);

int drsa_amd_drsa_fused_supported(int d, int K);
int drsa_amd_drsa_fused_step(const float* A, const float* C, int64_t N, int d, int K, const float* gs,
                             int64_t N_total, const float* U, float* U_out, float* f_out, float* gs_out, void* ws,
                             size_t ws_size, void* stream);

int drsa_amd_drsa_fused_step_counted(const float* A, const float* C, int64_t N, int d, int K, const float* gs,
                                     int64_t N_total, const float* U, float* U_out, float* f_traj, int* counter,
                                     float* gs_out, void* ws, size_t ws_size, void* stream);
int drsa_amd_drsa_finish_counted(const float* gs, int64_t N_total, int d, int K, const float* U, float* U_out,
                                 float* f_traj, int* counter, void* stream);

int drsa_amd_drsa_step(const float* A, const float* C, int64_t N, int d, int K, const float* U,
                       float* U_out, float* f_out, void* workspace, size_t workspace_bytes, void* stream);

int drsa_amd_drsa_objective(const float* A, const float* C, int64_t N, int d, int K, const float* U,
                            float* f_out, void* workspace, size_t workspace_bytes, void* stream);

int drsa_amd_drsa_run(const float* A, const float* C, int64_t N, int d, int K, float* U_io, float* U_tmp,
                      int steps, float* f_traj, int* counter, void* workspace, size_t workspace_bytes,
                      int use_graph, void* stream);

int drsa_amd_drsa_coop_status(const void* workspace, int64_t N, int d, int K, int* status_out, void* stream);

int drsa_amd_drsa_any_supported(int d, int K);
size_t drsa_amd_drsa_any_slab_floats(int d, int K);
size_t drsa_amd_drsa_any_workspace_bytes(int64_t N, int d, int K);
int drsa_amd_drsa_any_partial(const float* A, const float* C, int64_t N, int d, int K, const float* U,
                              float* gs_out, void* workspace, size_t workspace_bytes, void* stream);
int drsa_amd_drsa_any_finish(const float* gs, int64_t N_total, int d, int K, const float* U, float* U_out,
                             float* f_out, int objective_only, int* iters_out, void* stream);
int drsa_amd_drsa_any_finish_counted(const float* gs, int64_t N_total, int d, int K, const float* U, float* U_out,
                                     float* f_traj, int* counter, void* stream);
int drsa_amd_drsa_any_step(const float* A, const float* C, int64_t N, int d, int K, const float* U,
                           float* U_out, float* f_out, void* workspace, size_t workspace_bytes, void* stream);
int drsa_amd_drsa_any_objective(const float* A, const float* C, int64_t N, int d, int K, const float* U,
                                float* f_out, void* workspace, size_t workspace_bytes, void* stream);
int drsa_amd_drsa_any_run(const float* A, const float* C, int64_t N, int d, int K, float* U_io, float* U_tmp,
                          int steps, float* f_traj, int* counter, void* workspace, size_t workspace_bytes,
                          int use_graph, void* stream);

int drsa_amd_debug_coop_spin_budget(long long ticks);

int drsa_amd_polar(const float* V, int d, float* U_out, int* iters_out, void* stream);

size_t drsa_amd_subspace_relevances_workspace_bytes(int64_t B, int64_t N, int d, int K);
int drsa_amd_subspace_relevances(const float* act, const float* ctx, int64_t B, int64_t N, int d, int K,
                                 const float* U, float* out, void* workspace, size_t workspace_bytes, void* stream);


size_t drsa_amd_prca_workspace_bytes(int64_t N, int d);

int drsa_amd_prca_partial(const float* A, const float* C, int64_t N, int d, float* slab, void* ws, size_t ws_bytes,
                          void* stream);

int drsa_amd_prca_finish(const float* slab, int64_t N_total, int d, float* M_out, void* stream);

size_t drsa_amd_syevj_workspace_bytes(int d);
int drsa_amd_syevj(const float* M, int d, float* w_out, float* V_out, int* sweeps_out, void* ws, size_t ws_bytes,
                   void* stream);



size_t drsa_amd_conv_weight_floats(int cin, int cout, int ng);

int drsa_amd_conv_fwd(const float* in, const float* wts, const float* bias, const float* den_map, float* out,
                      uint8_t* out_amax, float* out_den, int B, int cin, int cout, int H, int W, int ng,
                      int pool, void* stream);

size_t drsa_amd_conv_weight_bf16_elems(int cin, int cout, int ng);
int drsa_amd_conv_fwd_bf16(const float* in, const uint16_t* wts, const float* bias, const float* den_map, float* out,
                           uint8_t* out_amax, float* out_den, int B, int cin, int cout, int H, int W, int ng,
                           int pool, void* stream);

int drsa_amd_conv_fwd_has_kernel(int cin, int cout, int W, int ng, int pool, int bf16);

int drsa_amd_conv_bwd(const float* g, const uint8_t* g_amax, const float* wts, const float* x, const float* den,
                      float* out, int Bq, int clones, int cin, int cout, int H, int W, int ng, int xmode,
                      int post, float eps, void* stream);

int drsa_amd_conv_bwd_bf16(const float* g, const uint8_t* g_amax, const uint16_t* wts, const float* x, const float* den,
                           float* out, int Bq, int clones, int cin, int cout, int H, int W, int ng, int xmode,
                           int post, float eps, void* stream);
int drsa_amd_conv_bwd_has_kernel_bf16(int cin, int cout, int W, int ng, int sparse);

int drsa_amd_conv_bwd_bf16_pw(const float* g, const uint8_t* g_amax, int pool_w, const uint16_t* wts, const float* x,
                              const float* den, float* out, int Bq, int clones, int cin, int cout, int H, int W,
                              int xmode, int post, float eps, void* stream);
int drsa_amd_conv_bwd_has_kernel_bf16_pw(int cin, int cout, int W, int pool_w);

int drsa_amd_conv_bwd_den_map(const float* g, const uint8_t* g_amax, int pool_w, const void* wts, int wts_bf16,
                              const float* x, const float* den_map, float* out, int Bq, int clones, int cin, int cout,
                              int H, int W, int ng, int xmode, float eps, void* stream);
int drsa_amd_conv_bwd_has_kernel_pw(int cin, int cout, int W, int ng, int pool_w);

int drsa_amd_convk_supported(int kh, int kw, int cin, int cout);
size_t drsa_amd_convk_weight_floats(int kh, int kw, int cin, int cout, int ng);
int drsa_amd_convk_fwd(const float* in, const float* wts, const float* bias, const float* den_map, float* out,
                       float* out_den, int B, int cin, int cout, int H, int W, int kh, int kw, int ng,
                       void* stream);
int drsa_amd_convk_bwd(const float* g, const float* wts, const float* x, const float* den, float* out, int Bq,
                       int clones, int cin, int cout, int H, int W, int kh, int kw, int ng, int xmode, int post,
                       float eps, void* stream);

int drsa_amd_conv_fwd_den_ring(const float* in, const float* wts, const float* bias, const float* den_map, float* out,
                               uint8_t* out_amax, float* den_ring, int B, int cout, int H, int W, int ng,
                               void* stream);
int drsa_amd_conv_bwd_den_ring(const float* g, const uint8_t* g_amax, const void* wts, int wts_bf16, const float* x,
                               const float* den_ring, const float* den_const4, float* out, int Bq, int clones, int cin,
                               int cout, int H, int W, int ng, int xmode, float eps, void* stream);

int drsa_amd_linear_fwd(const float* x, const float* W, const float* bias, float* z_out, float* relu_out, int M,
                        int N, int K, void* stream);

int drsa_amd_linear_bwd(const float* R, const int* seed_cls, int one_hot, const float* z, int relu_mask, int rule_eps,
                        float eps, const float* W, const float* x, int xmode, const float* den, int post,
                        float eps_post, float* out, int M, int Nout, int Kin, void* stream);

int drsa_amd_linear_rule_fwd(const float* x, const float* W, const float* Wp, const float* Wn, const float* bias,
                             const float* bias_p, const float* bias_n, float* z_out, float* relu_out, float* den_p,
                             float* den_n, int x_signed, int M, int N, int K, void* stream);
int drsa_amd_linear_rule_bwd(const float* R, const int* seed_cls, int one_hot, const float* z, int relu_mask,
                             const float* den_p, const float* den_n, int den_bcast, int zsign, float eps,
                             const float* Wp, const float* Wn, const float* x, int xmul, int x_signed,
                             const float* den, int post, float eps_post, float* out, int M, int Nout, int Kin,
                             void* stream);

int drsa_amd_projection_residual(const float* U, int d, float* P, void* stream);

int drsa_amd_projection_fwd(const float* a, const float* U, const float* P, float* h, float* ap, float* pooled,
                            uint8_t* amax, int B, int D, int H, int W, int pool, void* stream);

int drsa_amd_projection_bwd(const float* gp, const uint8_t* amax, const float* ap, const float* h, const float* a,
                            const float* den, const float* U, const float* P, float* G, int B, int D, int H, int W,
                            int K, float eps_proj, float eps_den, int fanout, void* stream);

int drsa_amd_projection_fwd_multi(const float* a, const float* U_tab, const float* P_tab, const int* u_row, int n_u,
                                  float* h, float* ap, float* pooled, uint8_t* amax, int B, int D, int H, int W,
                                  int pool, void* stream);
int drsa_amd_projection_bwd_multi(const float* gp, const uint8_t* amax, const float* ap, const float* h,
                                  const float* a, const float* den, const float* U_tab, const float* P_tab,
                                  const int* u_row, int n_u, float* G, int B, int D, int H, int W, int K,
                                  float eps_proj, float eps_den, int fanout, void* stream);

int drsa_amd_ab_split(const float* g, const float* den_p, const float* den_n, float* gp, float* gn, int Bq,
                      int clones, int64_t n, float eps, void* stream);
int drsa_amd_ab_combine(const float* pos, const float* neg, float alpha, float beta, const float* x, const float* den,
                        float* out, int Bq, int clones, int64_t n, int post, float eps, void* stream);

int drsa_amd_relevance_post(const float* R, const float* x, const float* den, float* out, int Bq, int clones,
                            int64_t n, int post, float eps, void* stream);

int drsa_amd_first_layer_bwd(const float* g, const uint8_t* amax, const float* w2, float* out, int Bq, int clones,
                             int C, int H, int W, void* stream);

int drsa_amd_first_layer_den(const float* w2, const float* b2, float* den, int C, int CI, int H, int W, void* stream);

int drsa_amd_first_layer_zbox_maps(const float* wp, const float* bp, const float* wn, const float* bn,
                                   const float* low_img, const float* high_img, float* zl, float* zh, int C, int H,
                                   int W, void* stream);
int drsa_amd_first_layer_zbox_den(const float* a, const uint8_t* amax, const float* zl, const float* zh, float* den,
                                  int B, int C, int H, int W, void* stream);
int drsa_amd_first_layer_zbox_bwd(const float* g, const uint8_t* amax, const float* wpn, const float* x,
                                  const float* low_img, const float* high_img, float* out, int Bq, int clones, int C,
                                  int H, int W, void* stream);

int drsa_amd_heatmap_sort(const float* hm, int B, int K, int HW, int std_from_sum, float* std_out, float* std_rel,
                          float* sub_out, float* rel, int64_t* mask, void* stream);

typedef struct drsa_amd_problem {
  const float* A;
  const float* C;
  int64_t N;
  int d;
  int K;
  float* U_io;
  float* U_tmp;
  float* f_traj;
  int* counter;
  void* ws;
  size_t ws_size;
  int dtype;
} drsa_amd_problem_t;

int drsa_amd_drsa_partial_bf16(const uint16_t* A, const uint16_t* C, int64_t N, int d, int K, const float* U,
                               float* gs_out, void* ws, size_t ws_size, void* stream);
int drsa_amd_drsa_partial_f16(const uint16_t* A, const uint16_t* C, int64_t N, int d, int K, const float* U,
                              float* gs_out, void* ws, size_t ws_size, void* stream);

int drsa_amd_drsa_run_multi(int P, const drsa_amd_problem_t* probs, int steps, int use_graph, void* stream);

int drsa_amd_drsa_run_batched(int P, const drsa_amd_problem_t* probs, int steps, int blocks, int use_graph,
                              void* stream);

int drsa_amd_logmel_smem_bytes(int n_fft, int hop, int n_mels, int width, int band_nnz);
int drsa_amd_logmel(const float* wav, int64_t n_songs, int64_t song_stride, int chunks_per_song, int64_t chunk_hop,
                    int chunk_len, int n_fft, int hop, int n_mels, int width, int frame0, const float* window,
                    const int* band_lo, const int* band_n, const int* band_off, const float* band_w, int band_nnz,
                    int peak_norm, int clamp, float clamp_min, float log_eps, float* out, void* stream);


int drsa_amd_maxpool_capture(const float* a, const float* den, float* y, uint8_t* amax, float* den_pooled, int B,
                             int C, int H, int W, int ph, int pw, void* stream);

int drsa_amd_relevance_unpool(const float* rel, const uint8_t* amax, int Bq, int clones, int C, int H, int W, int ph,
                              int pw, float* out, void* stream);

int drsa_amd_avgpool_fwd(const float* a, float* y, int B, int C, int H, int W, int ph, int pw, void* stream);

int drsa_amd_avgpool_bwd(const float* R_y, const float* y, const float* a, const float* den, int den_bcast, int rule,
                         float eps_pool, float eps_conv, float* g, float* rel_full, int Bq, int clones, int C, int H,
                         int W, int ph, int pw, void* stream);

int drsa_amd_drsa_vectors(const float* act, const float* rel, const uint8_t* rel_amax, const int* idx, int B, int C,
                          int H, int W, int ph, int pw, int L, int layout, float* A_out, float* C_out, void* stream);

size_t drsa_amd_normalize_workspace_bytes(void);
int drsa_amd_normalize_vectors(const float* v, int64_t n, int d, float* out, void* ws, size_t ws_bytes, void* stream);

int drsa_amd_normalize_sumsq(const float* v, int64_t n, void* ws, size_t ws_bytes, double* sum_out, void* stream);
int drsa_amd_normalize_scale(const float* v, int64_t n, int d, const double* sums, int nsums, int64_t n_total,
                             float* out, void* stream);


int drsa_amd_stft_mel_phase(const float* wav, int64_t n_chunks, int64_t chunk_stride, int chunk_len, int n_fft,
                            int hop, int n_mels, int width, int frame0, int power, const float* window,
                            const int* band_lo, const int* band_n, const int* band_off, const float* band_w,
                            int band_nnz, int peak_norm, float* mel, float* X, void* stream);

int drsa_amd_heatmap_mask(const float* heatmaps, int64_t n_maps, int H, int W, int group, int rank_first,
                          int rank_rest, const float* taps, int k, float* mask, void* stream);

int drsa_amd_istft_envelope(const float* window_host, int n_fft, int hop, int width, float* envelope_host);

int drsa_amd_mel_to_audio(const float* mel, const float* X, const float* mask, int64_t n_src, int C, int n_fft,
                          int hop, int n_mels, int width, int power, const float* window, const float* pinv_t,
                          const float* envelope, float* audio, void* stream);

int drsa_amd_audio_normalize(float* audio, int64_t n_audio, int len, const float* wav, int64_t wav_stride,
                             int wav_len, int C, void* stream);


int drsa_amd_mel_relevance_to_stft(const float* relevance, const float* mel, const float* X, int64_t n_src, int C,
                                   int n_mels, int width, int n_freq, const int* bin_lo, const int* bin_n,
                                   const int* bin_off, const float* bin_w, int bin_nnz, float eps, float* out,
                                   void* stream);

int drsa_amd_heatmap_mask_large(const float* heatmaps, int64_t n_maps, int H, int W, int group, int rank_first,
                                int rank_rest, const float* taps, int k, float* mask, void* stream);

int drsa_amd_stft_mask_to_audio(const float* X, const float* mask, int64_t n_src, int C, int n_fft, int hop,
                                int width, const float* window, const float* envelope, float* audio, void* stream);

#ifdef __cplusplus
}
#endif
#endif
```

Before: 115,300 explained samples/s.

## Process two relevance clones per workgroup in fp32 conv backward

Adds a clone-pair variant of the fp32 small-chunk 3x3 conv backward kernel in which each workgroup stages and computes two clones (DRSA subspace copies) of the same sample. The clones share the weights in LDS, the x/den epilogue loads and the tile setup, and the grid's batch dimension is halved. It is enabled by default for dense inputs when the clone count is even. In exchange it doubles halo and epilogue LDS and the per-wave accumulators, which can lower occupancy, and it halves the number of workgroups.

Measured after the change: 115,300 explained samples/s (median of 2 runs). Within noise of the previous version (-0.0%).

```diff
diff --git a/drsa_audio_amd/_capi.py b/drsa_audio_amd/_capi.py
--- a/drsa_audio_amd/_capi.py
+++ b/drsa_audio_amd/_capi.py
@@ -69,6 +69,7 @@
                                          _i32, _i32, _f32, _vp]),
     "drsa_amd_conv_bwd_has_kernel_pw": (_i32, [_i32, _i32, _i32, _i32, _i32]),
     "drsa_amd_conv_bwd_has_kernel_bf16_pw": (_i32, [_i32, _i32, _i32, _i32]),
+    "drsa_amd_conv_bwd_clones_per_wg": (_i32, [_i32, _i32, _i32, _i32, _i32, _i32, _i32, _i32]),
     "drsa_amd_conv_bwd_bf16_pw": (_i32, [_fp, _vp, _i32, _vp, _fp, _fp, _fp, _i32, _i32, _i32, _i32, _i32, _i32,
                                          _i32, _i32, _f32, _vp]),
     "drsa_amd_conv_bwd_has_kernel_bf16": (_i32, [_i32, _i32, _i32, _i32, _i32]),
diff --git a/drsa_audio_amd/csrc/conv_bwd_b.hip b/drsa_audio_amd/csrc/conv_bwd_b.hip
--- a/drsa_audio_amd/csrc/conv_bwd_b.hip
+++ b/drsa_audio_amd/csrc/conv_bwd_b.hip
@@ -7,9 +7,21 @@
 #define DRSA_CONV_CIC_BWD64_32 8
 #endif
 
+#if DRSA_CONV_PAIR_SPARSE
+#define PAIR_SPARSE(CIN, COUT) , CONV_ENTRY_PAIR(CIN, COUT, drsa_conv::A_POOLSPARSE)
+#else
+#define PAIR_SPARSE(CIN, COUT)
+#endif
+#if DRSA_CONV_PAIR_DENSE
+#define PAIR_DENSE(CIN, COUT) , CONV_ENTRY_PAIR(CIN, COUT, drsa_conv::A_DENSE)
+#else
+#define PAIR_DENSE(CIN, COUT)
+#endif
+
 CONV_TABLE(kTableBwdB,
     BWD_SET(64, 32, DRSA_CONV_CIC_BWD64_32),
-    BWD_SET(32, 32, DRSA_CONV_CIC_BWD32))
+    BWD_SET(32, 32, DRSA_CONV_CIC_BWD32)
+    PAIR_SPARSE(64, 32) PAIR_SPARSE(32, 32) PAIR_DENSE(64, 32) PAIR_DENSE(32, 32))
 
 #ifdef DRSA_CONV_STAMP
 extern "C" int drsa_amd_debug_conv_stamps(void* buf) {
diff --git a/drsa_audio_amd/csrc/lrp_conv.hip b/drsa_audio_amd/csrc/lrp_conv.hip
--- a/drsa_audio_amd/csrc/lrp_conv.hip
+++ b/drsa_audio_amd/csrc/lrp_conv.hip
@@ -22,13 +22,13 @@
 
 int pad32(int c) { return (c + 31) / 32 * 32; }
 
-const Entry* find(int cin_p, int cout_p, int W, int ng, int amode, int epi, int et = 0, int pw = 2) {
+const Entry* find(int cin_p, int cout_p, int W, int ng, int amode, int epi, int et = 0, int pw = 2, int cp = 1) {
   const int wide = W >= kWideW;
   for (const drsa_conv::Table* t : kTables)
     for (int i = 0; i < t->n; ++i) {
       const Entry& e = t->entries[i];
       if (e.cin_p == cin_p && e.cout_p == cout_p && e.ng == ng && e.amode == amode && e.epi == epi && e.et == et &&
-          e.pw == pw && e.wide == wide)
+          e.pw == pw && e.wide == wide && e.cp == cp)
         return &e;
     }
   return nullptr;
@@ -55,7 +55,7 @@
   const Entry* e = small_tile(e0, args.H, args.W, batch);
   DRSA_SMEM(e->fn, e->lds);
   const int tiles = ((args.H + e->th - 1) / e->th) * ((args.W + e->tw - 1) / e->tw);
-  hipLaunchKernelGGL(e->fn, dim3(tiles, batch), dim3(kThreads), e->lds, s, args);
+  hipLaunchKernelGGL(e->fn, dim3(tiles, batch / e->cp), dim3(kThreads), e->lds, s, args);
   DRSA_LAUNCH_CHECK();
   return DRSA_OK;
 }
@@ -69,6 +69,13 @@
 
 const Entry* find_bwd(int cin, int cout, int W, int ng, int sparse, int bf16, int pool_w) {
   return find(pad32(cin), pad32(cout), W, ng, sparse ? A_POOLSPARSE : A_DENSE, EPI_BWD, bf16 ? 1 : 0, pool_w);
+}
+
+const Entry* pick_bwd(int cin, int cout, int W, int ng, int sparse, int bf16, int pool_w, int clones) {
+  const Entry* e = find_bwd(cin, cout, W, ng, sparse, bf16, pool_w);
+  if (!e || bf16 || clones < 2 || clones % 2 != 0) return e;
+  const Entry* p = find(pad32(cin), pad32(cout), W, ng, sparse ? A_POOLSPARSE : A_DENSE, EPI_BWD, 0, pool_w, 2);
+  return p ? p : e;
 }
 
 int no_kernel(const char* entry, int cin, int cout, int W, int ng, int sparse, int bf16, const char* pool_key, int pool) {
@@ -141,7 +148,7 @@
   DRSA_REQUIRE(c.xmode == XM_NONE || c.x, "%s: xmode needs x", n);
   DRSA_REQUIRE(c.post == POST_NONE || (c.x && (c.den || c.post == POST_MASK)), "%s: POST_DIV needs x and den", n);
   const int sparse = c.g_amax != nullptr;
-  const Entry* e = find_bwd(c.cin, c.cout, c.W, c.ng, sparse, c.bf16, c.pool_w);
+  const Entry* e = pick_bwd(c.cin, c.cout, c.W, c.ng, sparse, c.bf16, c.pool_w, c.clones);
   if (!e) return no_kernel(n, c.cin, c.cout, c.W, c.ng, sparse, c.bf16, "pool_w", c.pool_w);
   ConvArgs a{};
   a.in = c.g; a.in_amax = c.g_amax; a.wts = reinterpret_cast<const float*>(c.wts); a.x = c.x; a.den = c.den;
@@ -181,6 +188,11 @@
 int drsa_amd_conv_bwd_has_kernel_bf16_pw(int cin, int cout, int W, int pool_w) {
   if (cin < 16 || (pool_w != 2 && pool_w != 4)) return 0;
   return find_bwd(cin, cout, W, 1, 1, 1, pool_w) != nullptr;
+}
+
+int drsa_amd_conv_bwd_clones_per_wg(int cin, int cout, int W, int ng, int sparse, int bf16, int pool_w, int clones) {
+  const Entry* e = pick_bwd(cin, cout, W, ng, sparse, bf16, pool_w, clones);
+  return e ? e->cp : 1;
 }
 
 int drsa_amd_conv_fwd(const float* in, const float* wts, const float* bias, const float* den_map, float* out,
diff --git a/drsa_audio_amd/csrc/lrp_conv_config.h b/drsa_audio_amd/csrc/lrp_conv_config.h
--- a/drsa_audio_amd/csrc/lrp_conv_config.h
+++ b/drsa_audio_amd/csrc/lrp_conv_config.h
@@ -43,6 +43,18 @@
 #ifndef DRSA_CONV_FWD128_TW
 #define DRSA_CONV_FWD128_TW 8
 #endif
+#ifndef DRSA_CONV_PAIR_SPARSE
+#define DRSA_CONV_PAIR_SPARSE 0
+#endif
+#ifndef DRSA_CONV_PAIR_DENSE
+#define DRSA_CONV_PAIR_DENSE 1
+#endif
+#ifndef DRSA_CONV_PAIR_TW
+#define DRSA_CONV_PAIR_TW 32
+#endif
+#ifndef DRSA_CONV_PAIR_PRE_D
+#define DRSA_CONV_PAIR_PRE_D 2
+#endif
 
 namespace drsa_conv {
 
@@ -77,10 +89,10 @@
   return r;
 }
 
-template <int CIN, int COUT, int TH, int TW, int MW, int CIC, int NG, int AMODE, int EPI, int ET = 0, int PW = 2>
+template <int CIN, int COUT, int TH, int TW, int MW, int CIC, int NG, int AMODE, int EPI, int ET = 0, int PW = 2, int CP = 1>
 struct ConvCfg {
   static constexpr int CIN_ = CIN, COUT_ = COUT, TH_ = TH, TW_ = TW, MW_ = MW, CIC_ = CIC, NG_ = NG;
-  static constexpr int AMODE_ = AMODE, EPI_ = EPI;
+  static constexpr int AMODE_ = AMODE, EPI_ = EPI, CP_ = CP;
   static constexpr bool BF = ET == 1;
   static constexpr int HY = TH + 2, HX = TW + 2;
   static constexpr int HXB = bf_stride(HX);
@@ -96,7 +108,8 @@
   static constexpr int NT = COUT / 32;
   static constexpr int WM = MT >= 4 ? 4 : MT;
   static constexpr int WN = (4 / WM) < NT ? (4 / WM) : NT;
-  static constexpr int MPW = MT / WM;
+  static constexpr int MPWC = MT / WM;
+  static constexpr int MPW = CP * MPWC;
   static constexpr int NPW = NT / WN;
   static constexpr int KC = 9 * CIC;
   static constexpr int KCP = round_up<KC, 2>();
@@ -106,8 +119,8 @@
   static constexpr int ES = (EPI == EPI_BWD && WN == 1) ? (SMALL_BWD ? DRSA_CONV_SMALL_ES : DRSA_CONV_BWD_ES) : 1;
   static constexpr int TCH = WN * 32 / ES;
   static constexpr size_t staging_floats =
-      BF ? bf_halo_floats + bf_w_floats : (size_t)CIC * PLANE + (size_t)NG * KCP * COUT;
-  static constexpr size_t epi_floats = (size_t)TCH * TH * TWP;
+      BF ? bf_halo_floats + bf_w_floats : (size_t)CP * CIC * PLANE + (size_t)NG * KCP * COUT;
+  static constexpr size_t epi_floats = (size_t)CP * TCH * TH * TWP;
   static constexpr size_t lds_floats = staging_floats > epi_floats ? staging_floats : epi_floats;
   static constexpr int WPE = BF ? (COUT <= 64 ? DRSA_CONV_BF_WPE : 1)
                              : (EPI == EPI_BWD && NG == 1) ? (SMALL_BWD ? DRSA_CONV_SMALL_WPE : DRSA_CONV_BWD_WPE)
@@ -126,6 +139,8 @@
                                                                   (ET == 1 || TW % 16 == 0)))),
                 "2x4 pool windows: the forward pool epilogue, or the backward's pool-sparse staging (fp32: "
                 "tiles of whole float4 cell groups)");
+  static_assert(CP == 1 || (CP == 2 && SMALL_BWD && ET == 0 && PW == 2 && WN == 1),
+                "clone pairs: the fp32 small-chunk backward only");
   static constexpr int PW_ = PW;
 };
 
diff --git a/drsa_audio_amd/csrc/lrp_conv_inst.h b/drsa_audio_amd/csrc/lrp_conv_inst.h
--- a/drsa_audio_amd/csrc/lrp_conv_inst.h
+++ b/drsa_audio_amd/csrc/lrp_conv_inst.h
@@ -15,6 +15,16 @@
   drsa_conv::conv_entry<CIN, COUT, TH, TW, MW, CIC, NG, AM, EP, ET, PW>(0)
 #define CONV_ENTRY_WIDE(CIN, COUT, TH, TW, MW, CIC, NG, AM, EP, ET, PW) \
   drsa_conv::conv_entry<CIN, COUT, TH, TW, MW, CIC, NG, AM, EP, ET, PW>(1)
+
+template <int CIN, int COUT, int AM>
+constexpr Entry conv_pair_entry() {
+  constexpr int TW = DRSA_CONV_PAIR_TW, TH = 128 / TW;
+  static_assert(TW == 32 || TW == 16, "pair tile: 4 x 32 or 8 x 16");
+  return Entry{CIN, COUT, TH, TW, 8, 8, 1, AM, EPI_BWD,
+               conv3x3_kernel<CIN, COUT, TH, TW, 8, 8, 1, AM, EPI_BWD, 0, 2, 2>,
+               ConvCfg<CIN, COUT, TH, TW, 8, 8, 1, AM, EPI_BWD, 0, 2, 2>::lds_floats * sizeof(float), 0, 2, 1, 2};
+}
+#define CONV_ENTRY_PAIR(CIN, COUT, AM) drsa_conv::conv_pair_entry<CIN, COUT, AM>()
 
 #define CONV_FAMILY(CIN, COUT, CIC, NG, AM, EP, ET, PW)                                             \
   CONV_ENTRY_WIDE(CIN, COUT, 8, drsa_conv::wide_tile_w(EP, ET, CIN, COUT),                          \
diff --git a/drsa_audio_amd/csrc/lrp_conv_kernel.h b/drsa_audio_amd/csrc/lrp_conv_kernel.h
--- a/drsa_audio_amd/csrc/lrp_conv_kernel.h
+++ b/drsa_audio_amd/csrc/lrp_conv_kernel.h
@@ -16,9 +16,10 @@
 
 __device__ const float g_zero_bias3[3 * 128] = {};
 
-template <int CIN, int COUT, int TH, int TW, int MW, int CIC, int NG, int AMODE, int EPI, int ET = 0, int PW = 2>
-__global__ __launch_bounds__(kThreads) __attribute__((amdgpu_waves_per_eu(ConvCfg<CIN, COUT, TH, TW, MW, CIC, NG, AMODE, EPI, ET, PW>::WPE))) void conv3x3_kernel(ConvArgs a) {
-  using Cfg = ConvCfg<CIN, COUT, TH, TW, MW, CIC, NG, AMODE, EPI, ET, PW>;
+template <int CIN, int COUT, int TH, int TW, int MW, int CIC, int NG, int AMODE, int EPI, int ET = 0, int PW = 2, int CP = 1>
+__global__ __launch_bounds__(kThreads) __attribute__((amdgpu_waves_per_eu(ConvCfg<CIN, COUT, TH, TW, MW, CIC, NG, AMODE, EPI, ET, PW, CP>::WPE))) void conv3x3_kernel(ConvArgs a) {
+  using Cfg = ConvCfg<CIN, COUT, TH, TW, MW, CIC, NG, AMODE, EPI, ET, PW, CP>;
+  static_assert(CP == 1 || EPI == EPI_BWD, "clone pairs are a backward tile");
   constexpr int HY = Cfg::HY, HX = Cfg::HX, RS = Cfg::RS, PLANE = Cfg::PLANE;
   constexpr int MTH = Cfg::MTH, MTW = Cfg::MTW, MTX = Cfg::MTX;
   constexpr int WM = Cfg::WM, MPW = Cfg::MPW, NPW = Cfg::NPW;
@@ -35,12 +36,12 @@
 #endif
   CONV_STAMP(0);
   float* halo = smem;
-  float* wl = smem + (Cfg::BF ? Cfg::bf_halo_floats : (size_t)CIC * PLANE);
+  float* wl = smem + (Cfg::BF ? Cfg::bf_halo_floats : (size_t)CP * CIC * PLANE);
 
   const int tid = threadIdx.x, lane = lane_id(), w = wave_id();
   const int H = a.H, W = a.W;
   const int tiles_x = (W + TW - 1) / TW;
-  const int tile_id = blockIdx.x, bq = blockIdx.y;
+  const int tile_id = blockIdx.x, bq = blockIdx.y * CP;
   const int ty0 = (tile_id / tiles_x) * TH;
   const int tx0 = (tile_id % tiles_x) * TW;
   const int bs = bq / a.clones;
@@ -51,11 +52,12 @@
   int pix_off[MPW], pix_y[MPW], pix_x[MPW];
 #pragma unroll
   for (int u = 0; u < MPW; ++u) {
-    const int mt = wm * MPW + u;
+    const int mt = wm * Cfg::MPWC + u % Cfg::MPWC;
     const int p = lane & 31, win = p >> 2, sub = p & 3;
     pix_y[u] = (mt / MTX) * MTH + 2 * (win / MW) + (sub >> 1);
     pix_x[u] = (mt % MTX) * MTW + 2 * (win % MW) + (sub & 1);
     pix_off[u] = Cfg::BF ? (h * HY + pix_y[u]) * Cfg::HXB + pix_x[u] : pix_y[u] * RS + pix_x[u] + XO;
+    if constexpr (CP > 1) pix_off[u] += (u / Cfg::MPWC) * CIC * PLANE;
   }
 
   f32x16 acc[NG][MPW][NPW];
@@ -76,6 +78,7 @@
   float* T = smem;
   constexpr int ES = Cfg::ES;
   static_assert(ES == 1 || ES == 2 || ES == 4, "epilogue split must be 1, 2 or 4");
+  constexpr int TCL = TCH * TH * TWP;
   auto stage = [&](int v, auto valfn, int sub = 0) {
     __syncthreads();
     if (active) {
@@ -84,10 +87,11 @@
 #pragma unroll
         for (int r = 0; r < 16; ++r) {
           const int cf = (r & 3) + 8 * (r >> 2) + 4 * h;
+          float* Tu = T + (CP > 1 ? (u / Cfg::MPWC) * TCL : 0);
           if constexpr (ES == 1) {
-            T[((wn * 32 + cf) * TH + pix_y[u]) * TWP + pix_x[u]] = valfn(u, r);
+            Tu[((wn * 32 + cf) * TH + pix_y[u]) * TWP + pix_x[u]] = valfn(u, r);
           } else {
-            if ((r >> (ES == 2 ? 3 : 2)) == sub) T[((cf - TCH * sub) * TH + pix_y[u]) * TWP + pix_x[u]] = valfn(u, r);
+            if ((r >> (ES == 2 ? 3 : 2)) == sub) Tu[((cf - TCH * sub) * TH + pix_y[u]) * TWP + pix_x[u]] = valfn(u, r);
           }
         }
     }
@@ -156,7 +160,24 @@
   };
   constexpr int kPreN = DRSA_CONV_PRE_N < V4T ? DRSA_CONV_PRE_N : V4T;
   float4 pre_x[V4T], pre_d[V4T];
-  if constexpr (EPI == EPI_BWD) {
+  constexpr int kPairD = CP > 1 ? (DRSA_CONV_PAIR_PRE_D < ES * V4T ? DRSA_CONV_PAIR_PRE_D : ES * V4T) : 0;
+  auto pair_dn = [](int sub) { return kPairD - sub * V4T < 0 ? 0 : kPairD - sub * V4T > V4T ? V4T : kPairD - sub * V4T; };
+  float4 pair_x[CP > 1 ? ES : 1][V4T], pair_d[CP > 1 ? ES : 1][V4T];
+  static_assert(CP == 1 || NPW == 1, "clone pairs: one n-tile per wave");
+  if constexpr (EPI == EPI_BWD && CP > 1) {
+    __syncthreads();
+    stg.store(halo, wl, tid);
+    __syncthreads();
+    CONV_STAMP(2 * Cfg::NCHUNK - 1);
+#pragma unroll
+    for (int sub = 0; sub < ES; ++sub) epi_loads(0, sub, pair_x[sub], pair_d[sub], true, false);
+#pragma unroll
+    for (int sub = 0; sub < ES; ++sub) epi_loads(0, sub, pair_x[sub], pair_d[sub], false, true, 0, pair_dn(sub));
+    if (active) mfma_chunk<Cfg, Cfg::PD>(halo, wl, pix_off, lane, wn, acc);
+    CONV_STAMP(2 * Cfg::NCHUNK);
+#pragma unroll
+    for (int sub = 0; sub < ES; ++sub) epi_loads(0, sub, pair_x[sub], pair_d[sub], false, true, pair_dn(sub), V4T);
+  } else if constexpr (EPI == EPI_BWD) {
     __syncthreads();
     if constexpr (Cfg::BF) stg.store(halo, wl, tid, ty0, tx0);
     else stg.store(halo, wl, tid);
@@ -378,6 +399,7 @@
         }
       }
     } else {
+     if constexpr (CP == 1) {
 #pragma unroll
      for (int sub = 0; sub < ES; ++sub) {
       float4 Rk[V4T], xk[V4T], dk[V4T];
@@ -458,6 +480,70 @@
         if (ok && pix_ok) *reinterpret_cast<float4*>(obase + (upix + (unsigned)coc * (unsigned)HW)) = R;
       }
      }
+     } else {
+#pragma unroll
+     for (int sub = 0; sub < ES; ++sub) {
+      float4 Rk[CP][V4T];
+      float4 (&xk)[V4T] = pair_x[sub], (&dk)[V4T] = pair_d[sub];
+      stage(v, [&](int u, int r) { return acc[0][u][v][r]; }, sub);
+      auto Tc = [&](int c) { return T + c * TCL; };
+      auto oc = [&](int c) { return obase + (size_t)c * a.cout * HW; };
+      if (a.xmode == XM_MUL && post_div) {
+#pragma unroll
+        for (int it = 0; it < V4T; ++it) {
+          const int cl = cl0 + it * CS;
+          const int co = gchs(cl, v, sub);
+          const bool ok = cl < TCH && co < a.cout;
+          const int clc = ok ? cl : 0, coc = ok ? co : 0;
+#pragma unroll
+          for (int c = 0; c < CP; ++c) {
+            const float4 t = *reinterpret_cast<const float4*>(Tc(c) + (clc * TH + py) * TWP + px);
+            const float4 x = xk[it], d = dk[it];
+            auto f = [&](float tt, float xx, float dd) {
+              const float q = div_nb(xx * tt, stab(dd, eps));
+              return (xx > 0.f) ? q : 0.f;
+            };
+            const float4 R = make_float4(f(t.x, x.x, d.x), f(t.y, x.y, d.y), f(t.z, x.z, d.z), f(t.w, x.w, d.w));
+            if (ok && pix_ok) *reinterpret_cast<float4*>(oc(c) + (upix + (unsigned)coc * (unsigned)HW)) = R;
+          }
+        }
+        continue;
+      }
+#pragma unroll
+      for (int it = 0; it < V4T; ++it) {
+        const int cl = cl0 + it * CS;
+        const int co = gchs(cl, v, sub);
+        const int clc = (cl < TCH && co < a.cout) ? cl : 0;
+#pragma unroll
+        for (int c = 0; c < CP; ++c) {
+          const float4 t = *reinterpret_cast<const float4*>(Tc(c) + (clc * TH + py) * TWP + px);
+          if (!need_x) xk[it] = make_float4(0.f, 0.f, 0.f, 0.f);
+          const float4 x = xk[it];
+          auto xm = [&](float xx) { const float m = split_x ? fmaxf(xx, 0.f) : xx; return mul_x ? m : 1.f; };
+          Rk[c][it] = make_float4(xm(x.x) * t.x, xm(x.y) * t.y, xm(x.z) * t.z, xm(x.w) * t.w);
+        }
+      }
+#pragma unroll
+      for (int it = 0; it < V4T; ++it) {
+        const int cl = cl0 + it * CS;
+        const int co = gchs(cl, v, sub);
+        const bool ok = cl < TCH && co < a.cout;
+        const int coc = ok ? co : 0;
+#pragma unroll
+        for (int c = 0; c < CP; ++c) {
+          float4 R = Rk[c][it];
+          const float4 x = xk[it], d = dk[it];
+          auto post = [&](float rr, float xx, float dd) {
+            const float q = div_nb(rr, stab(dd, eps));
+            const float y = post_div ? q : rr;
+            return (post_any && !(xx > 0.f)) ? 0.f : y;
+          };
+          R = make_float4(post(R.x, x.x, d.x), post(R.y, x.y, d.y), post(R.z, x.z, d.z), post(R.w, x.w, d.w));
+          if (ok && pix_ok) *reinterpret_cast<float4*>(oc(c) + (upix + (unsigned)coc * (unsigned)HW)) = R;
+        }
+      }
+     }
+     }
     }
   }
 #ifdef DRSA_CONV_STAMP
diff --git a/drsa_audio_amd/csrc/lrp_conv_stage.h b/drsa_audio_amd/csrc/lrp_conv_stage.h
--- a/drsa_audio_amd/csrc/lrp_conv_stage.h
+++ b/drsa_audio_amd/csrc/lrp_conv_stage.h
@@ -11,11 +11,13 @@
   static constexpr int NG = Cfg::NG_, HY = Cfg::HY, HX = Cfg::HX, RS = Cfg::RS, PLANE = Cfg::PLANE;
   static constexpr int KC = Cfg::KC, KCP = Cfg::KCP;
   static constexpr bool DENSE = Cfg::AMODE_ == A_DENSE;
+  static constexpr int CP = Cfg::CP_;
   static constexpr int Q4 = TW / 4, DROWS = CIC * HY;
-  static constexpr int DI = (DROWS * Q4 + NT_ - 1) / NT_, DH = (DROWS * 2 + NT_ - 1) / NT_;
+  static constexpr int DI = (CP * DROWS * Q4 + NT_ - 1) / NT_, DH = (CP * DROWS * 2 + NT_ - 1) / NT_;
   static constexpr int CY = TH / 2 + 2, CX = TW / 2 + 2, Q8 = TW / 8 > 0 ? TW / 8 : 1, SROWS = CIC * CY;
-  static constexpr int SI = (SROWS * Q8 + NT_ - 1) / NT_, SH = (SROWS * 2 + NT_ - 1) / NT_;
+  static constexpr int SI = (CP * SROWS * Q8 + NT_ - 1) / NT_, SH = (CP * SROWS * 2 + NT_ - 1) / NT_;
   static constexpr bool P4 = !DENSE && Cfg::PW_ == 4;
+  static_assert(CP == 1 || !P4, "clone pairs: dense or 2x2-pool-sparse g");
   static constexpr int Q16 = TW / 16 > 0 ? TW / 16 : 1;
   static constexpr int SI4 = (SROWS * Q16 + NT_ - 1) / NT_;
   static constexpr int NI = DENSE ? DI : P4 ? SI4 : SI, NH = DENSE ? DH : SH;
@@ -31,6 +33,8 @@
     const int W4 = W >> 2;
     const float* __restrict__ inb = a.in + (size_t)bq * a.cin * (DENSE ? H * W : H2 * (P4 ? W4 : W2));
     const uint8_t* __restrict__ amb = DENSE ? nullptr : a.in_amax + (size_t)bs * a.cin * H2 * (P4 ? W4 : W2);
+    const unsigned cstride = (unsigned)a.cin * (unsigned)(DENSE ? H * W : H2 * W2);
+    auto gp = [&](int o, int cl) { return CP > 1 ? inb + ((unsigned)o + (unsigned)cl * cstride) : inb + o; };
     if constexpr (P4) {
       const int qy0 = (ty0 >> 1) - 1, cx0 = tx0 >> 2;
 #pragma unroll
@@ -64,28 +68,30 @@
 #pragma unroll
         for (int it = 0; it < DI; ++it) {
           const int i = tid + it * NT_;
-          const int row = i / Q4, q = i % Q4;
+          const int rw = i / Q4, q = i % Q4;
+          const int cl = CP > 1 && i < CP * DROWS * Q4 ? rw / DROWS : 0, row = rw - cl * DROWS;
           const int ci = row / HY, hy = row % HY;
           const int gy = ty0 - 1 + hy, gx = tx0 + 4 * q, c = c0 + ci;
-          const bool ok = i < DROWS * Q4 && gy >= 0 && gy < H && c < a.cin && gx < W;
+          const bool ok = i < CP * DROWS * Q4 && gy >= 0 && gy < H && c < a.cin && gx < W;
           const int o = ok ? (c * H + gy) * W + gx : 0;
-          const float4 v = *reinterpret_cast<const float4*>(inb + o);
+          const float4 v = *reinterpret_cast<const float4*>(gp(o, cl));
           st_i[it] = ok ? v : make_float4(0.f, 0.f, 0.f, 0.f);
         }
       } else {
 #pragma unroll
         for (int it = 0; it < DI; ++it) {
           const int i = tid + it * NT_;
-          const int row = i / Q4, q = i % Q4;
+          const int rw = i / Q4, q = i % Q4;
+          const int cl = CP > 1 && i < CP * DROWS * Q4 ? rw / DROWS : 0, row = rw - cl * DROWS;
           const int ci = row / HY, hy = row % HY;
           const int gy = ty0 - 1 + hy, gx = tx0 + 4 * q, c = c0 + ci;
-          const bool rok = i < DROWS * Q4 && gy >= 0 && gy < H && c < a.cin;
+          const bool rok = i < CP * DROWS * Q4 && gy >= 0 && gy < H && c < a.cin;
           float vv[4];
 #pragma unroll
           for (int e = 0; e < 4; ++e) {
             const bool ok = rok && gx + e < W;
             const int o = ok ? (c * H + gy) * W + gx + e : 0;
-            const float v = inb[o];
+            const float v = *gp(o, cl);
             vv[e] = ok ? v : 0.f;
           }
           st_i[it] = make_float4(vv[0], vv[1], vv[2], vv[3]);
@@ -94,12 +100,13 @@
 #pragma unroll
       for (int it = 0; it < DH; ++it) {
         const int i = tid + it * NT_;
-        const int row = i >> 1, side = i & 1;
+        const int rw = i >> 1, side = i & 1;
+        const int cl = CP > 1 && i < CP * DROWS * 2 ? rw / DROWS : 0, row = rw - cl * DROWS;
         const int ci = row / HY, hy = row % HY;
         const int gy = ty0 - 1 + hy, gx = side ? tx0 + TW : tx0 - 1, c = c0 + ci;
-        const bool ok = i < DROWS * 2 && gy >= 0 && gy < H && gx >= 0 && gx < W && c < a.cin;
+        const bool ok = i < CP * DROWS * 2 && gy >= 0 && gy < H && gx >= 0 && gx < W && c < a.cin;
         const int o = ok ? (c * H + gy) * W + gx : 0;
-        const float v = inb[o];
+        const float v = *gp(o, cl);
         st_h[it] = ok ? v : 0.f;
       }
     } else {
@@ -108,12 +115,13 @@
 #pragma unroll
         for (int it = 0; it < SI; ++it) {
           const int i = tid + it * NT_;
-          const int row = i / Q8, q = i % Q8;
+          const int rw = i / Q8, q = i % Q8;
+          const int cl = CP > 1 && i < CP * SROWS * Q8 ? rw / SROWS : 0, row = rw - cl * SROWS;
           const int ci = row / CY, ry = row % CY;
           const int cy = qy0 + ry, cx = qx0 + 1 + 4 * q, c = c0 + ci;
-          const bool ok = i < SROWS * Q8 && 4 * q < TW / 2 && cy >= 0 && cy < H2 && c < a.cin && cx < W2;
+          const bool ok = i < CP * SROWS * Q8 && 4 * q < TW / 2 && cy >= 0 && cy < H2 && c < a.cin && cx < W2;
           const int o = ok ? (c * H2 + cy) * W2 + cx : 0;
-          const float4 v = *reinterpret_cast<const float4*>(inb + o);
+          const float4 v = *reinterpret_cast<const float4*>(gp(o, cl));
           const uint32_t am = *reinterpret_cast<const uint32_t*>(amb + o);
           st_i[it] = ok ? v : make_float4(0.f, 0.f, 0.f, 0.f);
           st_ia[it] = ok ? am : 0x04040404u;
@@ -122,17 +130,18 @@
 #pragma unroll
         for (int it = 0; it < SI; ++it) {
           const int i = tid + it * NT_;
-          const int row = i / Q8, q = i % Q8;
+          const int rw = i / Q8, q = i % Q8;
+          const int cl = CP > 1 && i < CP * SROWS * Q8 ? rw / SROWS : 0, row = rw - cl * SROWS;
           const int ci = row / CY, ry = row % CY;
           const int cy = qy0 + ry, cx = qx0 + 1 + 4 * q, c = c0 + ci;
-          const bool rok = i < SROWS * Q8 && 4 * q < TW / 2 && cy >= 0 && cy < H2 && c < a.cin;
+          const bool rok = i < CP * SROWS * Q8 && 4 * q < TW / 2 && cy >= 0 && cy < H2 && c < a.cin;
           float vv[4];
           uint32_t aa = 0;
 #pragma unroll
           for (int e = 0; e < 4; ++e) {
             const bool ok = rok && cx + e < W2 && 4 * q + e < TW / 2;
             const int o = ok ? (c * H2 + cy) * W2 + cx + e : 0;
-            const float v = inb[o];
+            const float v = *gp(o, cl);
             const uint32_t am = amb[o];
             vv[e] = ok ? v : 0.f;
             aa |= (ok ? am : 4u) << (8 * e);
@@ -144,12 +153,13 @@
 #pragma unroll
       for (int it = 0; it < SH; ++it) {
         const int i = tid + it * NT_;
-        const int row = i >> 1, side = i & 1;
+        const int rw = i >> 1, side = i & 1;
+        const int cl = CP > 1 && i < CP * SROWS * 2 ? rw / SROWS : 0, row = rw - cl * SROWS;
         const int ci = row / CY, ry = row % CY;
         const int cy = qy0 + ry, cx = side ? qx0 + CX - 1 : qx0, c = c0 + ci;
-        const bool ok = i < SROWS * 2 && cy >= 0 && cy < H2 && cx >= 0 && cx < W2 && c < a.cin;
+        const bool ok = i < CP * SROWS * 2 && cy >= 0 && cy < H2 && cx >= 0 && cx < W2 && c < a.cin;
         const int o = ok ? (c * H2 + cy) * W2 + cx : 0;
-        const float v = inb[o];
+        const float v = *gp(o, cl);
         const int am = (int)amb[o];
         st_h[it] = ok ? v : 0.f;
         st_ha[it] = ok ? am : 4;
@@ -208,7 +218,7 @@
 #pragma unroll
       for (int it = 0; it < DI; ++it) {
         const int i = tid + it * NT_;
-        if (i < DROWS * Q4) {
+        if (i < CP * DROWS * Q4) {
           const int row = i / Q4, q = i % Q4;
           const int ci = row / HY, hy = row % HY;
           *reinterpret_cast<float4*>(halo + ci * PLANE + hy * RS + 1 + XO + 4 * q) = st_i[it];
@@ -217,7 +227,7 @@
 #pragma unroll
       for (int it = 0; it < DH; ++it) {
         const int i = tid + it * NT_;
-        if (i < DROWS * 2) {
+        if (i < CP * DROWS * 2) {
           const int row = i >> 1, side = i & 1;
           const int ci = row / HY, hy = row % HY;
           halo[ci * PLANE + hy * RS + (side ? HX - 1 : 0) + XO] = st_h[it];
@@ -228,7 +238,7 @@
       for (int it = 0; it < SI; ++it) {
         const int i = tid + it * NT_;
         const int q = i % Q8;
-        if (i < SROWS * Q8 && 4 * q < TW / 2) {
+        if (i < CP * SROWS * Q8 && 4 * q < TW / 2) {
           const int row = i / Q8;
           const int ci = row / CY, ry = row % CY;
           const float vv[4] = {st_i[it].x, st_i[it].y, st_i[it].z, st_i[it].w};
@@ -240,7 +250,7 @@
 #pragma unroll
       for (int it = 0; it < SH; ++it) {
         const int i = tid + it * NT_;
-        if (i < SROWS * 2) {
+        if (i < CP * SROWS * 2) {
           const int row = i >> 1, side = i & 1;
           put_cell(halo, row / CY, row % CY, side ? CX - 1 : 0, st_h[it], st_ha[it]);
         }
diff --git a/drsa_audio_amd/csrc/lrp_conv_table.h b/drsa_audio_amd/csrc/lrp_conv_table.h
--- a/drsa_audio_amd/csrc/lrp_conv_table.h
+++ b/drsa_audio_amd/csrc/lrp_conv_table.h
@@ -13,6 +13,7 @@
   int et = 0;
   int pw = 2;
   int wide = 0;
+  int cp = 1;
 };
 
 struct Table {
diff --git a/include/drsa_amd.h b/include/drsa_amd.h
--- a/include/drsa_amd.h
+++ b/include/drsa_amd.h
@@ -116,6 +116,7 @@
                               const float* den, float* out, int Bq, int clones, int cin, int cout, int H, int W,
                               int xmode, int post, float eps, void* stream);
 int drsa_amd_conv_bwd_has_kernel_bf16_pw(int cin, int cout, int W, int pool_w);
+int drsa_amd_conv_bwd_clones_per_wg(int cin, int cout, int W, int ng, int sparse, int bf16, int pool_w, int clones);
 
 int drsa_amd_conv_bwd_den_map(const float* g, const uint8_t* g_amax, int pool_w, const void* wts, int wts_bf16,
                               const float* x, const float* den_map, float* out, int Bq, int clones, int cin, int cout,
```
